# Azure/gpu-provisioner

Hardware: AMD Instinct MI355X
Metric: nodeclaims_per_min (higher is better)
Workload: dtype n/a; 1 GPU; model=MI355X NodeClaim provisioning (karpenter CloudProvider contract), vm_sku=Standard_ND128isr_MI355X_v6, concurrent_nodeclaims=8, cloud=in-memory fake AKS, zero latency (BASELINE config #1), apiserver=in-memory, server-side CRD validation on, cycle=create→Launched→Registered→Initialized(amd.com/gpu)→delete→gone, parallelism=single

## Files before the change

### gpu_provisioner_amd/fake/apiserver.py

```python
from __future__ import annotations

import asyncio
import os
from collections import deque
from collections import defaultdict
from typing import Any, AsyncIterator, Callable, Optional

from ..kube import objects as ko
from ..kube.client import (
    ADDED,
    DELETED,
    MODIFIED,
    AlreadyExistsError,
    APIError,
    ConflictError,
    GoneError,
    InvalidError,
    KubeClient,
    LabelSelector,
    NotFoundError,
    json_merge_patch,
    match_field_selector,
    merge_patch_owned,
)

_WATCH_HISTORY = 4096
_WATCH_BROKEN = "__WATCH_BROKEN__"
_EVENT_CAP = 20000

_native_revstore = None
if os.environ.get("GPU_PROVISIONER_PURE_PYTHON") != "1":
    try:
        from .._native import _revstore as _native_revstore
    except ImportError:
        _native_revstore = None
NATIVE_REVSTORE = _native_revstore is not None
if NATIVE_REVSTORE:
    _native_revstore.set_helpers(ko.uuid4_str, ko.now_rfc3339)

_SELECTABLE_FIELDS = {
    ("v1", "Pod"): {
        "spec.nodeName",
        "spec.schedulerName",
        "spec.restartPolicy",
        "spec.serviceAccountName",
        "spec.hostNetwork",
        "status.phase",
        "status.podIP",
        "status.nominatedNodeName",
    },
    ("v1", "Node"): {"spec.unschedulable"},
    ("v1", "Namespace"): {"status.phase", "name"},
    ("v1", "Secret"): {"type"},
    ("v1", "Event"): {
        "involvedObject.kind",
        "involvedObject.namespace",
        "involvedObject.name",
        "involvedObject.uid",
        "involvedObject.apiVersion",
        "involvedObject.resourceVersion",
        "involvedObject.fieldPath",
        "reason",
        "reportingComponent",
        "source",
        "type",
    },
}
_GENERIC_FIELDS = {"metadata.name", "metadata.namespace"}


def validate_field_selector(api_version: str, kind: str, selector: str) -> None:
    if not selector:
        return
    allowed = _GENERIC_FIELDS | _SELECTABLE_FIELDS.get((api_version, kind), set())
    for part in selector.split(","):
        part = part.strip()
        if not part:
            continue
        key = part.split("!=" if "!=" in part else "=", 1)[0].strip()
        if key not in allowed:
            raise InvalidError(f"field label not supported: {key}")


def _key(namespace: str, name: str) -> tuple:
    return (namespace or "", name)


def _gvk(api_version: str, kind: str) -> tuple:
    return (api_version, kind)


class InMemoryAPIServer:

    def __init__(self):
        self._store: dict = defaultdict(dict)
        self._rv = 0
        self._native = _native_revstore
        self._event_cap = _EVENT_CAP
        self._lock = asyncio.Lock()
        self._watchers: list = []
        self._history: deque = deque(maxlen=_WATCH_HISTORY)
        self.reactors: list = []
        self.validators: dict = {}
        self.eviction_reactor: Optional[Callable] = None
        self.evictions: list = []


    def _next_rv(self) -> str:
        self._rv += 1
        return str(self._rv)

    def _fire_reactors(self, verb: str, gvk: tuple, payload: Any) -> None:
        for r in list(self.reactors):
            err = r(verb, gvk, payload)
            if err is not None:
                raise err

    def _broadcast(self, gvk: tuple, event_type: str, obj: dict) -> None:
        self._history.append((self._rv, gvk, event_type, obj))
        for wgvk, queue in self._watchers:
            if wgvk == gvk:
                queue.put_nowait((event_type, obj))

    def _bump(self, obj: dict) -> None:
        obj["metadata"]["resourceVersion"] = self._next_rv()

    def _validate(self, gvk: tuple, new: dict, old: Optional[dict]) -> None:
        fn = self.validators.get(gvk)
        if fn is None:
            return
        errs = fn(new, old)
        if errs:
            raise InvalidError(
                f"{gvk[1]} {ko.name_of(new)} is invalid: " + "; ".join(errs[:5])
            )


    async def get(self, api_version: str, kind: str, name: str, namespace: str) -> dict:
        async with self._lock:
            gvk = (api_version, kind)
            if self.reactors:
                self._fire_reactors("get", gvk, name)
            if self._native is not None:
                out = self._native.get(self._store[gvk], namespace, name)
                if out is not NotImplemented:
                    return out
            obj = self._store[gvk].get(_key(namespace, name))
            if obj is None:
                raise NotFoundError(f"{kind} {namespace}/{name} not found")
            return ko.deep_copy(obj)

    async def list(
        self,
        api_version: str,
        kind: str,
        namespace: str,
        label_selector: str,
        field_selector: str,
    ) -> tuple:
        async with self._lock:
            gvk = _gvk(api_version, kind)
            validate_field_selector(api_version, kind, field_selector)
            self._fire_reactors("list", gvk, None)
            sel = LabelSelector.parse(label_selector) if label_selector else None
            out = []
            for (ns, _), obj in self._store[gvk].items():
                if namespace and ns != namespace:
                    continue
                if sel and not sel.matches(ko.labels_of(obj)):
                    continue
                if not match_field_selector(obj, field_selector):
                    continue
                out.append(ko.deep_copy(obj))
            return out, str(self._peek_rv())

    def _peek_rv(self) -> int:
        return self._rv

    async def create(self, obj: dict) -> dict:
        async with self._lock:
            api_version, kind = obj.get("apiVersion", ""), obj.get("kind", "")
            if not api_version or not kind or not ko.name_of(obj):
                raise InvalidError("apiVersion, kind and metadata.name are required")
            gvk = (api_version, kind)
            if self.reactors:
                self._fire_reactors("create", gvk, obj)
            if self._native is not None:
                out = self._native.create(
                    self, gvk, self._store[gvk], obj, self.validators.get(gvk), self._event_cap
                )
                if out is not NotImplemented:
                    return out
            key = _key(ko.namespace_of(obj), ko.name_of(obj))
            if key in self._store[gvk]:
                raise AlreadyExistsError(f"{kind} {key[0]}/{key[1]} already exists")
            stored = ko.deep_copy(obj)
            m = ko.meta(stored)
            m["uid"] = m.get("uid") or ko.uuid4_str()
            m["creationTimestamp"] = m.get("creationTimestamp") or ko.now_rfc3339()
            m["generation"] = 1
            self._validate(gvk, stored, None)
            self._bump(stored)
            self._store[gvk][key] = stored
            if kind == "Event" and len(self._store[gvk]) > self._event_cap:
                drop = next(iter(self._store[gvk]))
                del self._store[gvk][drop]
            self._broadcast(gvk, ADDED, stored)
            return ko.deep_copy(stored)

    async def update(self, obj: dict, subresource: str = "") -> dict:
        async with self._lock:
            api_version, kind = obj.get("apiVersion", ""), obj.get("kind", "")
            gvk = (api_version, kind)
            if self.reactors:
                self._fire_reactors("update", gvk, obj)
            if self._native is not None:
                out = self._native.update(
                    self, gvk, self._store[gvk], obj, subresource, self.validators.get(gvk)
                )
                if out is not NotImplemented:
                    return out
            key = _key(ko.namespace_of(obj), ko.name_of(obj))
            cur = self._store[gvk].get(key)
            if cur is None:
                raise NotFoundError(f"{kind} {key[0]}/{key[1]} not found")
            rv = obj.get("metadata", {}).get("resourceVersion")
            if rv and rv != cur["metadata"]["resourceVersion"]:
                raise ConflictError(
                    f"{kind} {key[1]}: resourceVersion mismatch ({rv} != {cur['metadata']['resourceVersion']})"
                )
            return self._apply_update(gvk, key, cur, obj, subresource)

    def _apply_update(
        self, gvk: tuple, key: tuple, cur: dict, obj: dict, subresource: str, owned: bool = False
    ) -> dict:
        if subresource == "status":
            stored = {**cur, "metadata": {**cur["metadata"]}}
            stored["status"] = ko.deep_copy(obj.get("status", {}))
        else:
            if ko.is_deleting(cur):
                added = set(ko.finalizers_of(obj)) - set(ko.finalizers_of(cur))
                if added:
                    raise InvalidError(
                        "metadata.finalizers: Forbidden: no new finalizers can "
                        f"be added if the object is being deleted (added: {sorted(added)})"
                    )
            new = obj if owned else ko.deep_copy(obj)
            new["status"] = cur.get("status", {})
            nm = ko.meta(new)
            cm = cur["metadata"]
            for f in ("uid", "creationTimestamp", "generation", "deletionTimestamp"):
                if f in cm:
                    nm[f] = cm[f]
                else:
                    nm.pop(f, None)
            ns, cs = new.get("spec"), cur.get("spec")
            if ns is cs:
                pass
            elif ns != cs:
                nm["generation"] = cm.get("generation", 1) + 1
            elif "spec" in new:
                new["spec"] = cs
            stored = new
        self._validate(gvk, stored, cur)
        self._bump(stored)
        if ko.is_deleting(stored) and not ko.finalizers_of(stored) and subresource != "status":
            del self._store[gvk][key]
            self._broadcast(gvk, DELETED, stored)
        else:
            self._store[gvk][key] = stored
            self._broadcast(gvk, MODIFIED, stored)
        return ko.deep_copy(stored)

    async def patch(
        self,
        api_version: str,
        kind: str,
        name: str,
        patch: dict,
        namespace: str,
        subresource: str,
    ) -> dict:
        async with self._lock:
            gvk = (api_version, kind)
            if self.reactors:
                self._fire_reactors("patch", gvk, name)
            if self._native is not None:
                out = self._native.patch(
                    self, gvk, self._store[gvk], namespace, name, patch, subresource,
                    self.validators.get(gvk),
                )
                if out is not NotImplemented:
                    return out
            key = _key(namespace, name)
            cur = self._store[gvk].get(key)
            if cur is None:
                raise NotFoundError(f"{kind} {namespace}/{name} not found")
            req_rv = (patch.get("metadata") or {}).get("resourceVersion")
            if req_rv and req_rv != cur["metadata"]["resourceVersion"]:
                raise ConflictError(
                    f"{kind} {name}: resourceVersion mismatch "
                    f"({req_rv} != {cur['metadata']['resourceVersion']})"
                )
            if subresource == "status":
                merged_status = json_merge_patch(cur.get("status", {}), patch.get("status", patch))
                return self._apply_update(gvk, key, cur, {"status": merged_status}, "status")
            merged = merge_patch_owned(cur, patch)
            merged.setdefault("metadata", {})["resourceVersion"] = cur["metadata"]["resourceVersion"]
            return self._apply_update(gvk, key, cur, merged, "", owned=True)

    async def delete(
        self,
        api_version: str,
        kind: str,
        name: str,
        namespace: str,
        uid_precondition: str = "",
        grace_period_seconds: Optional[int] = None,
    ) -> None:
        async with self._lock:
            gvk = (api_version, kind)
            if self.reactors:
                self._fire_reactors("delete", gvk, name)
            if self._native is not None:
                out = self._native.delete(
                    self, gvk, self._store[gvk], namespace, name, uid_precondition
                )
                if out is not NotImplemented:
                    return out
            key = _key(namespace, name)
            cur = self._store[gvk].get(key)
            if cur is None:
                raise NotFoundError(f"{kind} {namespace}/{name} not found")
            if uid_precondition and ko.uid_of(cur) != uid_precondition:
                raise ConflictError(f"{kind} {name}: uid precondition failed")
            if ko.finalizers_of(cur):
                if not ko.is_deleting(cur):
                    stored = {**cur, "metadata": {**cur["metadata"]}}
                    ko.meta(stored)["deletionTimestamp"] = ko.now_rfc3339()
                    self._bump(stored)
                    self._store[gvk][key] = stored
                    self._broadcast(gvk, MODIFIED, stored)
                return
            stored = {**cur, "metadata": {**cur["metadata"]}}
            ko.meta(stored)["deletionTimestamp"] = ko.now_rfc3339()
            self._bump(stored)
            del self._store[gvk][key]
            self._broadcast(gvk, DELETED, stored)

    async def evict(self, pod: dict, grace_period_seconds: Optional[int]) -> None:
        async with self._lock:
            if self.eviction_reactor is not None:
                err = self.eviction_reactor(pod)
                if err is not None:
                    raise err
            gvk = _gvk("v1", "Pod")
            key = _key(ko.namespace_of(pod), ko.name_of(pod))
            cur = self._store[gvk].get(key)
            if cur is None:
                raise NotFoundError(f"Pod {key[0]}/{key[1]} not found")
            self.evictions.append(key)
            stored = ko.deep_copy(cur)
            ko.meta(stored)["deletionTimestamp"] = ko.now_rfc3339()
            self._bump(stored)
            if ko.finalizers_of(cur):
                self._store[gvk][key] = stored
                self._broadcast(gvk, MODIFIED, stored)
            else:
                del self._store[gvk][key]
                self._broadcast(gvk, DELETED, stored)

    def subscribe(self, api_version: str, kind: str, resource_version: str) -> tuple:
        gvk = _gvk(api_version, kind)
        queue: asyncio.Queue = asyncio.Queue()
        if resource_version:
            rv = int(resource_version)
            if self._history:
                oldest = self._history[0][0]
                if rv + 1 < oldest and any(True for _ in self._store[gvk]):
                    raise GoneError(f"resourceVersion {rv} too old")
            for erv, egvk, etype, eobj in self._history:
                if egvk == gvk and erv > rv:
                    queue.put_nowait((etype, ko.deep_copy(eobj)))
        entry = (gvk, queue)
        self._watchers.append(entry)

        def unsubscribe():
            try:
                self._watchers.remove(entry)
            except ValueError:
                pass

        return queue, unsubscribe

    def break_watches(self) -> int:
        broken = 0
        for _, queue in list(self._watchers):
            queue.put_nowait((_WATCH_BROKEN, None))
            broken += 1
        return broken


class InMemoryClient(KubeClient):

    def __init__(self, server: InMemoryAPIServer):
        self.server = server

    async def get(self, api_version: str, kind: str, name: str, namespace: str = "") -> dict:
        return await self.server.get(api_version, kind, name, namespace)

    async def list(
        self,
        api_version: str,
        kind: str,
        namespace: str = "",
        label_selector: str = "",
        field_selector: str = "",
    ) -> list:
        items, _rv = await self.server.list(api_version, kind, namespace, label_selector, field_selector)
        return items

    async def list_with_rv(
        self,
        api_version: str,
        kind: str,
        namespace: str = "",
        label_selector: str = "",
        field_selector: str = "",
    ) -> tuple:
        return await self.server.list(api_version, kind, namespace, label_selector, field_selector)

    async def create(self, obj: dict) -> dict:
        return await self.server.create(obj)

    async def update(self, obj: dict) -> dict:
        return await self.server.update(obj)

    async def update_status(self, obj: dict) -> dict:
        return await self.server.update(obj, subresource="status")

    async def patch(
        self,
        api_version: str,
        kind: str,
        name: str,
        patch: dict,
        namespace: str = "",
        subresource: str = "",
    ) -> dict:
        return await self.server.patch(api_version, kind, name, patch, namespace, subresource)

    async def delete(
        self,
        api_version: str,
        kind: str,
        name: str,
        namespace: str = "",
        uid_precondition: str = "",
        grace_period_seconds: Optional[int] = None,
    ) -> None:
        await self.server.delete(
            api_version, kind, name, namespace, uid_precondition, grace_period_seconds
        )

    async def watch(
        self,
        api_version: str,
        kind: str,
        namespace: str = "",
        resource_version: str = "",
        label_selector: str = "",
    ) -> AsyncIterator[tuple]:
        queue, unsubscribe = self.server.subscribe(api_version, kind, resource_version)
        sel = LabelSelector.parse(label_selector) if label_selector else None
        try:
            while True:
                event_type, obj = await queue.get()
                if event_type == _WATCH_BROKEN:
                    raise APIError("watch stream broken")
                if namespace and ko.namespace_of(obj) != namespace:
                    continue
                if sel and not sel.matches(ko.labels_of(obj)):
                    continue
                yield event_type, obj
        finally:
            unsubscribe()

    async def evict(self, pod: dict, grace_period_seconds: Optional[int] = None) -> None:
        await self.server.evict(pod, grace_period_seconds)
```

### gpu_provisioner_amd/kube/crdschema.py

```python
from __future__ import annotations

import re
from typing import Optional

from .objects import _native_jsontree

_native_valid = _native_jsontree.crd_valid if _native_jsontree is not None else None


def _compile_schema(schema: dict, cache: Optional[dict] = None) -> dict:
    if cache is None:
        cache = {}
    sid = id(schema)
    if sid in cache:
        return cache[sid]
    out = dict(schema)
    cache[sid] = out
    if "pattern" in out:
        out["_pattern_re"] = re.compile(out["pattern"])
    if "enum" in out:
        out["_enum_set"] = frozenset(out["enum"])
    if "properties" in out:
        out["properties"] = {
            k: _compile_schema(v, cache) for k, v in out["properties"].items()
        }
    if isinstance(out.get("items"), dict):
        out["items"] = _compile_schema(out["items"], cache)
    if isinstance(out.get("additionalProperties"), dict):
        out["additionalProperties"] = _compile_schema(out["additionalProperties"], cache)
    for branch in ("anyOf", "oneOf", "allOf"):
        if branch in out:
            out[branch] = [_compile_schema(b, cache) for b in out[branch]]
    return out


def validate(obj, schema: dict, path: str = "$") -> list:
    errs: list = []
    _validate(obj, schema, (path,), errs)
    return errs


def _render(parts: tuple) -> str:
    return "".join(parts)


def _validate(obj, schema: dict, path: tuple, errs: list) -> None:
    t = schema.get("type")
    if t == "object" or ("properties" in schema and t is None):
        if not isinstance(obj, dict):
            errs.append(f"{_render(path)}: expected object, got {type(obj).__name__}")
            return
        props = schema.get("properties")
        ap = schema.get("additionalProperties")
        if props:
            extra_ok = schema.get("x-kubernetes-preserve-unknown-fields") or ap is not None
            for k, v in obj.items():
                sub = props.get(k)
                if sub is not None:
                    _validate(v, sub, path + (".", k), errs)
                elif isinstance(ap, dict):
                    _validate(v, ap, path + (".", k), errs)
                elif not extra_ok:
                    errs.append(f"{_render(path)}.{k}: unknown field")
        elif isinstance(ap, dict):
            for k, v in obj.items():
                _validate(v, ap, path + (".", k), errs)
        for req in schema.get("required", ()):
            if req not in obj:
                errs.append(f"{_render(path)}.{req}: required field missing")
    elif t == "array":
        if not isinstance(obj, list):
            errs.append(f"{_render(path)}: expected array, got {type(obj).__name__}")
            return
        if "maxItems" in schema and len(obj) > schema["maxItems"]:
            errs.append(
                f"{_render(path)}: {len(obj)} items exceeds maxItems {schema['maxItems']}"
            )
        items = schema.get("items")
        if items:
            for i, item in enumerate(obj):
                _validate(item, items, path + (f"[{i}]",), errs)
    elif t == "string":
        if not isinstance(obj, str):
            errs.append(f"{_render(path)}: expected string, got {type(obj).__name__}")
        else:
            enum_set = schema.get("_enum_set")
            if enum_set is not None:
                if obj not in enum_set:
                    errs.append(f"{_render(path)}: {obj!r} not in enum {schema['enum']}")
            elif "enum" in schema and obj not in schema["enum"]:
                errs.append(f"{_render(path)}: {obj!r} not in enum {schema['enum']}")
            pat = schema.get("_pattern_re")
            if pat is not None:
                if pat.search(obj) is None:
                    errs.append(
                        f"{_render(path)}: {obj!r} does not match pattern {schema['pattern']!r}"
                    )
            elif "pattern" in schema and re.search(schema["pattern"], obj) is None:
                errs.append(
                    f"{_render(path)}: {obj!r} does not match pattern {schema['pattern']!r}"
                )
            if "maxLength" in schema and len(obj) > schema["maxLength"]:
                errs.append(
                    f"{_render(path)}: length {len(obj)} exceeds maxLength {schema['maxLength']}"
                )
            if "minLength" in schema and len(obj) < schema["minLength"]:
                errs.append(
                    f"{_render(path)}: length {len(obj)} below minLength {schema['minLength']}"
                )
    elif t == "integer":
        if not isinstance(obj, int) or isinstance(obj, bool):
            errs.append(f"{_render(path)}: expected integer, got {type(obj).__name__}")
        else:
            if "minimum" in schema and obj < schema["minimum"]:
                errs.append(f"{_render(path)}: {obj} below minimum {schema['minimum']}")
            if "maximum" in schema and obj > schema["maximum"]:
                errs.append(f"{_render(path)}: {obj} above maximum {schema['maximum']}")
    elif t == "boolean":
        if not isinstance(obj, bool):
            errs.append(f"{_render(path)}: expected boolean, got {type(obj).__name__}")
    if "anyOf" in schema:
        branch_errs: list = []
        ok = False
        for b in schema["anyOf"]:
            merged = b
            if b.get("type") == "string" and any(
                f in schema for f in ("pattern", "_pattern_re", "maxLength", "minLength", "enum")
            ):
                merged = {**b}
                for f in ("pattern", "_pattern_re", "maxLength", "minLength", "enum", "_enum_set"):
                    if f in schema:
                        merged[f] = schema[f]
            be: list = []
            _validate(obj, merged, path, be)
            if not be:
                ok = True
                break
            if not branch_errs:
                branch_errs = be
        if not ok:
            errs.append(
                f"{_render(path)}: no anyOf branch matched ({'; '.join(branch_errs[:1])})"
            )


_MISSING = object()


def _validate_changed(new, old, schema: dict, path: str, errs: list) -> None:
    if new is old:
        return
    props = schema.get("properties")
    if isinstance(new, dict) and isinstance(old, dict) and props is not None:
        ap = schema.get("additionalProperties")
        extra_ok = schema.get("x-kubernetes-preserve-unknown-fields") or ap is not None
        for k, v in new.items():
            sub = props.get(k)
            if sub is None and isinstance(ap, dict):
                sub = ap
            if sub is None:
                if props and not extra_ok:
                    errs.append(f"{path}.{k}: unknown field")
                continue
            ov = old.get(k, _MISSING)
            if ov is _MISSING:
                _validate(v, sub, (path, ".", k), errs)
            else:
                _validate_changed(v, ov, sub, f"{path}.{k}", errs)
        for req in schema.get("required", ()):
            if req not in new:
                errs.append(f"{path}.{req}: required field missing")
        return
    items = schema.get("items")
    if isinstance(new, list) and isinstance(old, list) and isinstance(items, dict):
        if "maxItems" in schema and len(new) > schema["maxItems"]:
            errs.append(f"{path}: {len(new)} items exceeds maxItems {schema['maxItems']}")
        for i, item in enumerate(new):
            if any(item is o or item == o for o in old):
                continue
            _validate(item, items, (path, f"[{i}]"), errs)
        return
    if new == old:
        return
    _validate(new, schema, (path,), errs)


def _apply_defaults(obj, schema: dict) -> None:
    if not isinstance(obj, dict):
        return
    for name, sub in (schema.get("properties") or {}).items():
        if name not in obj and "default" in sub:
            obj[name] = sub["default"]
        if name in obj:
            if isinstance(obj[name], dict):
                _apply_defaults(obj[name], sub)
            elif isinstance(obj[name], list) and isinstance(sub.get("items"), dict):
                for item in obj[name]:
                    _apply_defaults(item, sub["items"])


class CRDValidator:

    def __init__(self, crd: dict):
        versions = crd["spec"]["versions"]
        assert len(versions) == 1
        self.schema = _compile_schema(versions[0]["schema"]["openAPIV3Schema"])
        spec_schema = self.schema.get("properties", {}).get("spec", {})
        self.spec_immutable = any(
            r.get("rule") == "self == oldSelf"
            for r in spec_schema.get("x-kubernetes-validations", [])
        )

    @classmethod
    def from_file(cls, path: str) -> "CRDValidator":
        import yaml

        return cls(next(yaml.safe_load_all(open(path))))

    def __call__(self, new: dict, old: Optional[dict]) -> list:
        if old is None:
            _apply_defaults(new, self.schema)
        if _native_valid is not None and _native_valid(
            self.schema, new, old, self.spec_immutable
        ):
            return []
        return self._violations(new, old)

    def _violations(self, new: dict, old: Optional[dict]) -> list:
        errs: list = []
        if old is None:
            errs += validate(new, self.schema)
        else:
            props = self.schema.get("properties", {})
            for key in ("spec", "status"):
                ns, olds = new.get(key), old.get(key)
                sub = props.get(key)
                if sub is not None and ns is not None:
                    _validate_changed(ns, olds, sub, f"$.{key}", errs)
            if self.spec_immutable:
                ns, olds = new.get("spec"), old.get("spec")
                if ns is not olds and ns != olds:
                    errs.append("$.spec: spec is immutable (CEL: self == oldSelf)")
        ref = (new.get("spec") or {}).get("nodeClassRef")
        if isinstance(ref, dict):
            for f in ("group", "kind", "name"):
                if f in ref and ref[f] == "":
                    errs.append(f"$.spec.nodeClassRef.{f}: may not be empty (CEL)")
        return errs
```

### native/jsontree.cpp

```cpp
#define PY_SSIZE_T_CLEAN
#include <Python.h>

#include "jsontree_walk.h"

namespace {

using jsontree_walk::copy_tree;
using jsontree_walk::merge;
using jsontree_walk::merge_owned;

PyObject* py_deep_copy(PyObject*, PyObject* obj) { return copy_tree(obj); }

PyObject* py_json_merge_patch(PyObject*, PyObject* const* args, Py_ssize_t nargs) {
    if (nargs != 2) {
        PyErr_SetString(PyExc_TypeError, "json_merge_patch(target, patch) takes 2 arguments");
        return nullptr;
    }
    return merge(args[0], args[1], false);
}

PyObject* str_metadata;

PyObject* py_merge_patch_owned(PyObject*, PyObject* const* args, Py_ssize_t nargs) {
    if (nargs != 2) {
        PyErr_SetString(PyExc_TypeError, "merge_patch_owned(cur, patch) takes 2 arguments");
        return nullptr;
    }
    return merge_owned(args[0], args[1], str_metadata);
}


struct Names {
    PyObject *type, *properties, *additionalProperties, *preserve, *required, *items,
        *maxItems, *enum_set, *enum_, *pattern_re, *pattern, *maxLength, *minLength,
        *minimum, *maximum, *anyOf, *search, *spec, *status, *nodeClassRef, *group,
        *kind, *name, *empty;
} S;

inline PyObject* sget(PyObject* schema, PyObject* key) {
    PyObject* v = PyDict_GetItemWithError(schema, key);
    if (v == nullptr) PyErr_Clear();
    return v;
}

inline PyObject* sget2(PyObject* schema, PyObject* overlay, PyObject* key) {
    if (overlay != nullptr) {
        PyObject* v = sget(overlay, key);
        if (v != nullptr) return v;
    }
    return sget(schema, key);
}

inline bool is_str(PyObject* o, const char* s) {
    return o != nullptr && PyUnicode_CheckExact(o) && PyUnicode_CompareWithASCIIString(o, s) == 0;
}

int len_cmp(Py_ssize_t n, PyObject* limit, int op) {
    PyObject* pn = PyLong_FromSsize_t(n);
    if (pn == nullptr) return -1;
    int r = PyObject_RichCompareBool(pn, limit, op);
    Py_DECREF(pn);
    return r;
}

int validate(PyObject* obj, PyObject* schema, PyObject* overlay);

int validate_changed(PyObject* nw, PyObject* old, PyObject* schema);

int check_required(PyObject* obj, PyObject* schema) {
    PyObject* req = sget(schema, S.required);
    if (req == nullptr) return 1;
    if (!PyList_CheckExact(req) && !PyTuple_CheckExact(req)) return 0;
    Py_ssize_t n = PySequence_Fast_GET_SIZE(req);
    for (Py_ssize_t i = 0; i < n; i++) {
        int has = PyDict_Contains(obj, PySequence_Fast_GET_ITEM(req, i));
        if (has <= 0) return has;
    }
    return 1;
}

int validate_string(PyObject* obj, PyObject* schema, PyObject* overlay) {
    if (!PyUnicode_Check(obj)) return 0;
    if (!PyUnicode_CheckExact(obj)) return 0;
    PyObject* enum_set = sget2(schema, overlay, S.enum_set);
    if (enum_set != nullptr && enum_set != Py_None) {
        int in = PySequence_Contains(enum_set, obj);
        if (in <= 0) return in;
    } else {
        PyObject* en = sget2(schema, overlay, S.enum_);
        if (en != nullptr) {
            int in = PySequence_Contains(en, obj);
            if (in <= 0) return in;
        }
    }
    PyObject* pat = sget2(schema, overlay, S.pattern_re);
    if (pat != nullptr && pat != Py_None) {
        PyObject* m = PyObject_CallMethodOneArg(pat, S.search, obj);
        if (m == nullptr) return -1;
        bool miss = m == Py_None;
        Py_DECREF(m);
        if (miss) return 0;
    } else if (sget2(schema, overlay, S.pattern) != nullptr) {
        return 0;
    }
    PyObject* lim = sget2(schema, overlay, S.maxLength);
    if (lim != nullptr) {
        int r = len_cmp(PyUnicode_GET_LENGTH(obj), lim, Py_GT);
        if (r != 0) return r < 0 ? -1 : 0;
    }
    lim = sget2(schema, overlay, S.minLength);
    if (lim != nullptr) {
        int r = len_cmp(PyUnicode_GET_LENGTH(obj), lim, Py_LT);
        if (r != 0) return r < 0 ? -1 : 0;
    }
    return 1;
}

int validate_object(PyObject* obj, PyObject* schema) {
    if (!PyDict_Check(obj)) return 0;
    if (!PyDict_CheckExact(obj)) return 0;
    PyObject* props = sget(schema, S.properties);
    PyObject* ap = sget(schema, S.additionalProperties);
    if (ap == Py_None) ap = nullptr;
    if (ap != nullptr && PyDict_Check(ap) && !PyDict_CheckExact(ap)) return 0;
    bool ap_schema = ap != nullptr && PyDict_CheckExact(ap);
    int props_true = props == nullptr ? 0 : PyObject_IsTrue(props);
    if (props_true < 0) return -1;
    if (props_true && !PyDict_CheckExact(props)) return 0;
    if (props_true || ap_schema) {
        bool extra_ok = ap != nullptr;
        if (props_true && !extra_ok) {
            PyObject* pu = sget(schema, S.preserve);
            int t = pu == nullptr ? 0 : PyObject_IsTrue(pu);
            if (t < 0) return -1;
            extra_ok = t != 0;
        }
        Py_ssize_t pos = 0;
        PyObject *k, *v;
        while (PyDict_Next(obj, &pos, &k, &v)) {
            PyObject* sub = nullptr;
            if (props_true) {
                sub = PyDict_GetItemWithError(props, k);
                if (sub == nullptr && PyErr_Occurred()) return -1;
                if (sub == Py_None) sub = nullptr;
            }
            if (sub == nullptr && ap_schema) sub = ap;
            if (sub == nullptr) {
                if (!extra_ok) return 0;
                continue;
            }
            if (!PyDict_CheckExact(sub)) return 0;
            int r = validate(v, sub, nullptr);
            if (r <= 0) return r;
        }
    }
    return check_required(obj, schema);
}

int validate_any_of(PyObject* obj, PyObject* schema, PyObject* branches) {
    if (!PyList_CheckExact(branches)) return 0;
    bool string_fields = sget(schema, S.pattern) || sget(schema, S.pattern_re) ||
                         sget(schema, S.maxLength) || sget(schema, S.minLength) ||
                         sget(schema, S.enum_);
    for (Py_ssize_t i = 0; i < PyList_GET_SIZE(branches); i++) {
        PyObject* b = PyList_GET_ITEM(branches, i);
        if (!PyDict_CheckExact(b)) return 0;
        PyObject* overlay = nullptr;
        if (string_fields && is_str(sget(b, S.type), "string")) overlay = schema;
        int r = validate(obj, b, overlay);
        if (r != 0) return r;
    }
    return 0;
}

int validate(PyObject* obj, PyObject* schema, PyObject* overlay) {
    if (Py_EnterRecursiveCall(" while validating against a CRD schema")) return -1;
    int r = 1;
    PyObject* t = sget(schema, S.type);
    if (t != nullptr && t != Py_None && !PyUnicode_CheckExact(t)) {
        r = 0;
    } else if (is_str(t, "object") ||
               ((t == nullptr || t == Py_None) && sget(schema, S.properties) != nullptr)) {
        r = validate_object(obj, schema);
    } else if (is_str(t, "array")) {
        if (!PyList_CheckExact(obj)) {
            r = 0;
        } else {
            PyObject* lim = sget(schema, S.maxItems);
            if (lim != nullptr) {
                int c = len_cmp(PyList_GET_SIZE(obj), lim, Py_GT);
                if (c != 0) r = c < 0 ? -1 : 0;
            }
            PyObject* items = sget(schema, S.items);
            int items_true = (r == 1 && items != nullptr) ? PyObject_IsTrue(items) : 0;
            if (items_true < 0) r = -1;
            if (r == 1 && items_true) {
                if (!PyDict_CheckExact(items)) r = 0;
                for (Py_ssize_t i = 0; r == 1 && i < PyList_GET_SIZE(obj); i++)
                    r = validate(PyList_GET_ITEM(obj, i), items, nullptr);
            }
        }
    } else if (is_str(t, "string")) {
        r = validate_string(obj, schema, overlay);
    } else if (is_str(t, "integer")) {
        if (!PyLong_Check(obj) || PyBool_Check(obj)) {
            r = 0;
        } else {
            PyObject* lim = sget(schema, S.minimum);
            if (lim != nullptr) {
                int c = PyObject_RichCompareBool(obj, lim, Py_LT);
                if (c != 0) r = c < 0 ? -1 : 0;
            }
            lim = sget(schema, S.maximum);
            if (r == 1 && lim != nullptr) {
                int c = PyObject_RichCompareBool(obj, lim, Py_GT);
                if (c != 0) r = c < 0 ? -1 : 0;
            }
        }
    } else if (is_str(t, "boolean")) {
        if (!PyBool_Check(obj)) r = 0;
    }
    if (r == 1) {
        PyObject* any_of = sget(schema, S.anyOf);
        if (any_of != nullptr)
            r = overlay != nullptr ? 0 : validate_any_of(obj, schema, any_of);
    }
    Py_LeaveRecursiveCall();
    return r;
}

int validate_changed(PyObject* nw, PyObject* old, PyObject* schema) {
    if (nw == old) return 1;
    if (Py_EnterRecursiveCall(" while validating against a CRD schema")) return -1;
    int r = 1;
    PyObject* props = sget(schema, S.properties);
    if (props == Py_None) props = nullptr;
    PyObject* items = sget(schema, S.items);
    if ((PyDict_Check(nw) && !PyDict_CheckExact(nw)) || (PyDict_Check(old) && !PyDict_CheckExact(old)) ||
        (PyList_Check(nw) && !PyList_CheckExact(nw)) || (PyList_Check(old) && !PyList_CheckExact(old)) ||
        (props != nullptr && !PyDict_CheckExact(props)) ||
        (items != nullptr && PyDict_Check(items) && !PyDict_CheckExact(items))) {
        r = 0;
    } else if (PyDict_CheckExact(nw) && PyDict_CheckExact(old) && props != nullptr) {
        PyObject* ap = sget(schema, S.additionalProperties);
        if (ap == Py_None) ap = nullptr;
        bool ap_schema = ap != nullptr && PyDict_CheckExact(ap);
        if (ap != nullptr && PyDict_Check(ap) && !ap_schema) r = 0;
        bool extra_ok = ap != nullptr;
        if (r == 1 && !extra_ok) {
            PyObject* pu = sget(schema, S.preserve);
            int t = pu == nullptr ? 0 : PyObject_IsTrue(pu);
            if (t < 0) r = -1;
            extra_ok = t > 0;
        }
        bool props_true = PyDict_GET_SIZE(props) > 0;
        Py_ssize_t pos = 0;
        PyObject *k, *v;
        while (r == 1 && PyDict_Next(nw, &pos, &k, &v)) {
            PyObject* sub = PyDict_GetItemWithError(props, k);
            if (sub == nullptr && PyErr_Occurred()) { r = -1; break; }
            if (sub == Py_None) sub = nullptr;
            if (sub == nullptr && ap_schema) sub = ap;
            if (sub == nullptr) {
                if (props_true && !extra_ok) r = 0;
                continue;
            }
            if (!PyDict_CheckExact(sub)) { r = 0; break; }
            PyObject* ov = PyDict_GetItemWithError(old, k);
            if (ov == nullptr && PyErr_Occurred()) { r = -1; break; }
            r = ov == nullptr ? validate(v, sub, nullptr) : validate_changed(v, ov, sub);
        }
        if (r == 1) r = check_required(nw, schema);
    } else if (PyList_CheckExact(nw) && PyList_CheckExact(old) && items != nullptr &&
               PyDict_CheckExact(items)) {
        PyObject* lim = sget(schema, S.maxItems);
        if (lim != nullptr) {
            int c = len_cmp(PyList_GET_SIZE(nw), lim, Py_GT);
            if (c != 0) r = c < 0 ? -1 : 0;
        }
        for (Py_ssize_t i = 0; r == 1 && i < PyList_GET_SIZE(nw); i++) {
            PyObject* item = PyList_GET_ITEM(nw, i);
            Py_INCREF(item);
            int seen = 0;
            for (Py_ssize_t j = 0; seen == 0 && j < PyList_GET_SIZE(old); j++) {
                PyObject* o = PyList_GET_ITEM(old, j);
                Py_INCREF(o);
                seen = PyObject_RichCompareBool(item, o, Py_EQ);
                Py_DECREF(o);
            }
            if (seen < 0) r = -1;
            else if (seen == 0) r = validate(item, items, nullptr);
            Py_DECREF(item);
        }
    } else {
        int eq = PyObject_RichCompareBool(nw, old, Py_EQ);
        if (eq < 0) r = -1;
        else if (eq == 0) r = validate(nw, schema, nullptr);
    }
    Py_LeaveRecursiveCall();
    return r;
}

int crd_valid(PyObject* schema, PyObject* nw, PyObject* old, bool spec_immutable) {
    if (!PyDict_CheckExact(schema) || !PyDict_CheckExact(nw)) return 0;
    PyObject* spec = sget(nw, S.spec);
    if (old == Py_None) {
        int r = validate(nw, schema, nullptr);
        if (r <= 0) return r;
    } else {
        if (!PyDict_CheckExact(old)) return 0;
        PyObject* props = sget(schema, S.properties);
        if (props != nullptr && !PyDict_CheckExact(props)) return 0;
        PyObject* keys[2] = {S.spec, S.status};
        for (PyObject* key : keys) {
            PyObject* ns = sget(nw, key);
            PyObject* olds = sget(old, key);
            PyObject* sub = props ? sget(props, key) : nullptr;
            if (sub == nullptr || sub == Py_None || ns == nullptr || ns == Py_None) continue;
            if (!PyDict_CheckExact(sub)) return 0;
            int r = validate_changed(ns, olds ? olds : Py_None, sub);
            if (r <= 0) return r;
        }
        if (spec_immutable) {
            PyObject* ns = spec ? spec : Py_None;
            PyObject* olds = sget(old, S.spec);
            if (olds == nullptr) olds = Py_None;
            if (ns != olds) {
                int ne = PyObject_RichCompareBool(ns, olds, Py_NE);
                if (ne != 0) return ne < 0 ? -1 : 0;
            }
        }
    }
    if (spec == nullptr) return 1;
    int spec_true = PyObject_IsTrue(spec);
    if (spec_true < 0) return -1;
    if (!spec_true) return 1;
    if (!PyDict_CheckExact(spec)) return 0;
    PyObject* ref = sget(spec, S.nodeClassRef);
    if (ref == nullptr || !PyDict_Check(ref)) return 1;
    if (!PyDict_CheckExact(ref)) return 0;
    PyObject* fields[3] = {S.group, S.kind, S.name};
    for (PyObject* f : fields) {
        PyObject* v = sget(ref, f);
        if (v == nullptr) continue;
        int eq = PyObject_RichCompareBool(v, S.empty, Py_EQ);
        if (eq != 0) return eq < 0 ? -1 : 0;
    }
    return 1;
}

PyObject* py_crd_valid(PyObject*, PyObject* const* args, Py_ssize_t nargs) {
    if (nargs != 4) {
        PyErr_SetString(PyExc_TypeError,
                        "crd_valid(schema, new, old_or_None, spec_immutable) takes 4 arguments");
        return nullptr;
    }
    int imm = PyObject_IsTrue(args[3]);
    if (imm < 0) return nullptr;
    int r = crd_valid(args[0], args[1], args[2], imm != 0);
    if (r < 0) {
        PyErr_Clear();
        r = 0;
    }
    return PyBool_FromLong(r);
}

PyMethodDef methods[] = {
    {"deep_copy", (PyCFunction)py_deep_copy, METH_O,
     "deep_copy(obj): copy exact dict/list recursively, share everything else."},
    {"json_merge_patch", (PyCFunction)(void (*)(void))py_json_merge_patch, METH_FASTCALL,
     "json_merge_patch(target, patch): RFC 7386 merge patch, returning a new dict."},
    {"merge_patch_owned", (PyCFunction)(void (*)(void))py_merge_patch_owned, METH_FASTCALL,
     "merge_patch_owned(cur, patch): == deep_copy(json_merge_patch(cur, patch)), "
     "sharing the subtrees of cur the patch does not touch."},
    {"crd_valid", (PyCFunction)(void (*)(void))py_crd_valid, METH_FASTCALL,
     "crd_valid(schema, new, old_or_None, spec_immutable): True when CRDValidator "
     "would report no violation."},
    {nullptr, nullptr, 0, nullptr},
};

PyModuleDef moduledef = {
    PyModuleDef_HEAD_INIT, "_jsontree",
    "Native JSON-tree copy, merge patch and CRD validation fast path.", -1, methods,
    nullptr, nullptr, nullptr, nullptr,
};

bool intern_names() {
    struct { PyObject** slot; const char* text; } table[] = {
        {&str_metadata, "metadata"},
        {&S.type, "type"},
        {&S.properties, "properties"},
        {&S.additionalProperties, "additionalProperties"},
        {&S.preserve, "x-kubernetes-preserve-unknown-fields"},
        {&S.required, "required"},
        {&S.items, "items"},
        {&S.maxItems, "maxItems"},
        {&S.enum_set, "_enum_set"},
        {&S.enum_, "enum"},
        {&S.pattern_re, "_pattern_re"},
        {&S.pattern, "pattern"},
        {&S.maxLength, "maxLength"},
        {&S.minLength, "minLength"},
        {&S.minimum, "minimum"},
        {&S.maximum, "maximum"},
        {&S.anyOf, "anyOf"},
        {&S.search, "search"},
        {&S.spec, "spec"},
        {&S.status, "status"},
        {&S.nodeClassRef, "nodeClassRef"},
        {&S.group, "group"},
        {&S.kind, "kind"},
        {&S.name, "name"},
        {&S.empty, ""},
    };
    for (auto& e : table) {
        *e.slot = PyUnicode_InternFromString(e.text);
        if (*e.slot == nullptr) return false;
    }
    return true;
}

}

PyMODINIT_FUNC PyInit__jsontree(void) {
    if (!intern_names()) return nullptr;
    return PyModule_Create(&moduledef);
}
```

### native/revstore.cpp

```cpp
#define PY_SSIZE_T_CLEAN
#include <Python.h>

#include <limits.h>

#include "jsontree_walk.h"

namespace {

using jsontree_walk::copy_tree;
using jsontree_walk::merge;
using jsontree_walk::merge_owned;

struct Names {
    PyObject *metadata, *name, *namespace_, *uid, *creationTimestamp, *generation,
        *deletionTimestamp, *finalizers, *resourceVersion, *spec, *status, *empty, *Event,
        *ADDED, *MODIFIED, *DELETED, *rv_attr, *history_attr, *watchers_attr, *append,
        *put_nowait;
} S;

PyObject* long_one;
PyObject* uuid4_str;
PyObject* now_rfc3339;

struct Ref {
    PyObject* p;
    explicit Ref(PyObject* o = nullptr) : p(o) {}
    ~Ref() { Py_XDECREF(p); }
    Ref(const Ref&) = delete;
    Ref& operator=(const Ref&) = delete;
    void reset(PyObject* o) { Py_XSETREF(p, o); }
    PyObject* release() {
        PyObject* o = p;
        p = nullptr;
        return o;
    }
    operator PyObject*() const { return p; }
};

inline PyObject* newref(PyObject* o) {
    Py_XINCREF(o);
    return o;
}

inline PyObject* miss() { Py_RETURN_NOTIMPLEMENTED; }

inline int look(PyObject* d, PyObject* key, PyObject** out) {
    *out = PyDict_GetItemWithError(d, key);
    if (*out != nullptr) return 1;
    return PyErr_Occurred() ? -1 : 0;
}

inline int truthy(PyObject* d, PyObject* key) {
    PyObject* v;
    int r = look(d, key, &v);
    if (r <= 0) return r;
    Ref hold(newref(v));
    return PyObject_IsTrue(v);
}

inline bool str_eq(PyObject* a, PyObject* b) {
    return a == b || PyUnicode_Compare(a, b) == 0;
}

PyObject* make_key(PyObject* ns, PyObject* name) {
    if (ns == nullptr || ns == Py_None) ns = S.empty;
    if (name == nullptr || !PyUnicode_CheckExact(ns) || !PyUnicode_CheckExact(name)) return nullptr;
    return PyTuple_Pack(2, ns, name);
}

int current(PyObject* bucket, PyObject* key, PyObject** cur, PyObject** cm) {
    int r = look(bucket, key, cur);
    if (r <= 0) return r;
    if (!PyDict_CheckExact(*cur)) return 0;
    r = look(*cur, S.metadata, cm);
    if (r == 1 && !PyDict_CheckExact(*cm)) return 0;
    return r;
}

int rv_precondition(PyObject* meta, PyObject* cm) {
    PyObject* want = nullptr;
    if (meta != nullptr && look(meta, S.resourceVersion, &want) < 0) return -1;
    if (want == nullptr || want == Py_None) return 1;
    if (!PyUnicode_CheckExact(want)) return 0;
    if (PyUnicode_GET_LENGTH(want) == 0) return 1;
    PyObject* have;
    int r = look(cm, S.resourceVersion, &have);
    if (r <= 0) return r;
    return PyUnicode_CheckExact(have) && str_eq(want, have);
}

int no_new_finalizers(PyObject* nm, PyObject* cm) {
    PyObject *nf, *cf;
    if (look(nm, S.finalizers, &nf) < 0 || look(cm, S.finalizers, &cf) < 0) return -1;
    if (nf == nullptr || nf == Py_None) return 1;
    if (cf == Py_None) cf = nullptr;
    if (!PyList_CheckExact(nf) || (cf != nullptr && !PyList_CheckExact(cf))) return 0;
    for (Py_ssize_t i = 0; i < PyList_GET_SIZE(nf); i++) {
        PyObject* f = PyList_GET_ITEM(nf, i);
        if (!PyUnicode_CheckExact(f)) return 0;
        bool found = false;
        for (Py_ssize_t j = 0; !found && cf != nullptr && j < PyList_GET_SIZE(cf); j++) {
            PyObject* c = PyList_GET_ITEM(cf, j);
            if (!PyUnicode_CheckExact(c)) return 0;
            found = str_eq(f, c);
        }
        if (!found) return 0;
    }
    return 1;
}

int valid(PyObject* validator, PyObject* nw, PyObject* old) {
    if (validator == Py_None) return 1;
    PyObject* args[2] = {nw, old};
    Ref errs(PyObject_Vectorcall(validator, args, 2, nullptr));
    if (errs == nullptr) return -1;
    int t = PyObject_IsTrue(errs);
    return t < 0 ? -1 : !t;
}


struct Sink {
    Ref append;
    Ref watchers;
    long long rv = 0;
};

int open_sink(PyObject* server, Sink& s) {
    Ref rv(PyObject_GetAttr(server, S.rv_attr));
    Ref hist(rv != nullptr ? PyObject_GetAttr(server, S.history_attr) : nullptr);
    if (hist != nullptr) s.append.reset(PyObject_GetAttr(hist, S.append));
    if (s.append != nullptr) s.watchers.reset(PyObject_GetAttr(server, S.watchers_attr));
    if (s.watchers == nullptr) {
        PyErr_Clear();
        return 0;
    }
    PyObject* ws = s.watchers.p;
    if (!PyLong_CheckExact(rv.p) || !PyList_CheckExact(ws)) return 0;
    int overflow = 0;
    s.rv = PyLong_AsLongLongAndOverflow(rv.p, &overflow);
    if (overflow || s.rv < 0 || s.rv == LLONG_MAX) return 0;
    for (Py_ssize_t i = 0; i < PyList_GET_SIZE(ws); i++) {
        PyObject* w = PyList_GET_ITEM(ws, i);
        if (!PyTuple_CheckExact(w) || PyTuple_GET_SIZE(w) != 2) return 0;
    }
    return 1;
}

int commit(PyObject* server, Sink& s, PyObject* gvk, PyObject* bucket, PyObject* key,
           PyObject* stored, PyObject* nm, PyObject* event_type, bool remove,
           Py_ssize_t cap = -1) {
    long long n = s.rv + 1;
    Ref rv_str(PyUnicode_FromFormat("%lld", n));
    Ref rv_int(PyLong_FromLongLong(n));
    if (rv_str == nullptr || rv_int == nullptr) return -1;
    Ref entry(PyTuple_Pack(4, (PyObject*)rv_int, gvk, event_type, stored));
    Ref event(PyTuple_Pack(2, event_type, stored));
    if (entry == nullptr || event == nullptr) return -1;
    if (PyDict_SetItem(nm, S.resourceVersion, rv_str) < 0) return -1;
    if (PyObject_SetAttr(server, S.rv_attr, rv_int) < 0) return -1;
    if ((remove ? PyDict_DelItem(bucket, key) : PyDict_SetItem(bucket, key, stored)) < 0) return -1;
    if (cap >= 0 && PyDict_GET_SIZE(bucket) > cap) {
        Py_ssize_t pos = 0;
        PyObject *k, *v;
        if (PyDict_Next(bucket, &pos, &k, &v)) {
            Ref oldest(newref(k));
            if (PyDict_DelItem(bucket, oldest) < 0) return -1;
        }
    }
    Ref appended(PyObject_CallOneArg(s.append, entry));
    if (appended == nullptr) return -1;
    PyObject* ws = s.watchers.p;
    for (Py_ssize_t i = 0; i < PyList_GET_SIZE(ws); i++) {
        PyObject* w = PyList_GET_ITEM(ws, i);
        if (!PyTuple_CheckExact(w) || PyTuple_GET_SIZE(w) != 2) continue;
        Ref hold(newref(w));
        int eq = PyObject_RichCompareBool(PyTuple_GET_ITEM(w, 0), gvk, Py_EQ);
        if (eq < 0) return -1;
        if (!eq) continue;
        Ref put(PyObject_CallMethodOneArg(PyTuple_GET_ITEM(w, 1), S.put_nowait, event));
        if (put == nullptr) return -1;
    }
    return 0;
}


enum Mode {
    STATUS,
    STATUS_OWNED,
    MAIN,
    MAIN_OWNED,
};

PyObject* apply_update(PyObject* server, PyObject* gvk, PyObject* bucket, PyObject* key,
                       PyObject* cur, PyObject* cm, PyObject* obj, Mode mode,
                       PyObject* validator) {
    Sink sink;
    if (!open_sink(server, sink)) return miss();
    Ref stored, meta_ref;
    bool remove = false;
    if (mode == STATUS || mode == STATUS_OWNED) {
        stored.reset(PyDict_Copy(cur));
        meta_ref.reset(PyDict_Copy(cm));
        if (stored == nullptr || meta_ref == nullptr) return nullptr;
        Ref status;
        if (mode == STATUS_OWNED) {
            status.reset(newref(obj));
        } else {
            PyObject* v;
            if (look(obj, S.status, &v) < 0) return nullptr;
            status.reset(v != nullptr ? copy_tree(v) : PyDict_New());
        }
        if (status == nullptr || PyDict_SetItem(stored, S.metadata, meta_ref) < 0 ||
            PyDict_SetItem(stored, S.status, status) < 0)
            return nullptr;
    } else {
        PyObject* om;
        int r = look(obj, S.metadata, &om);
        if (r < 0) return nullptr;
        if (r == 0 || !PyDict_CheckExact(om)) return miss();
        int deleting = truthy(cm, S.deletionTimestamp);
        if (deleting < 0) return nullptr;
        if (deleting) {
            r = no_new_finalizers(om, cm);
            if (r < 0) return nullptr;
            if (r == 0) return miss();
        }
        stored.reset(mode == MAIN_OWNED ? newref(obj) : copy_tree(obj));
        if (stored == nullptr) return nullptr;
        PyObject* v;
        if (look(cur, S.status, &v) < 0) return nullptr;
        Ref status(v != nullptr ? newref(v) : PyDict_New());
        if (status == nullptr || PyDict_SetItem(stored, S.status, status) < 0) return nullptr;
        if (look(stored, S.metadata, &v) <= 0) return nullptr;
        meta_ref.reset(newref(v));
        PyObject* fixed[4] = {S.uid, S.creationTimestamp, S.generation, S.deletionTimestamp};
        for (PyObject* f : fixed) {
            if (look(cm, f, &v) < 0) return nullptr;
            if (v != nullptr) {
                if (PyDict_SetItem(meta_ref, f, v) < 0) return nullptr;
            } else {
                int has = PyDict_Contains(meta_ref, f);
                if (has < 0 || (has && PyDict_DelItem(meta_ref, f) < 0)) return nullptr;
            }
        }
        PyObject *ns, *cs;
        if (look(stored, S.spec, &ns) < 0 || look(cur, S.spec, &cs) < 0) return nullptr;
        PyObject* a = ns != nullptr ? ns : Py_None;
        PyObject* b = cs != nullptr ? cs : Py_None;
        if (a != b) {
            int ne = PyObject_RichCompareBool(a, b, Py_NE);
            if (ne < 0) return nullptr;
            if (ne) {
                PyObject* gen;
                if (look(cm, S.generation, &gen) < 0) return nullptr;
                if (gen == nullptr) gen = long_one;
                if (!PyLong_CheckExact(gen)) return miss();
                Ref next(PyNumber_Add(gen, long_one));
                if (next == nullptr || PyDict_SetItem(meta_ref, S.generation, next) < 0) return nullptr;
            } else if (ns != nullptr && cs != nullptr) {
                if (PyDict_SetItem(stored, S.spec, cs) < 0) return nullptr;
            }
        }
    }
    int ok = valid(validator, stored, cur);
    if (ok < 0) return nullptr;
    if (!ok) return miss();
    if (mode == MAIN || mode == MAIN_OWNED) {
        int deleting = truthy(meta_ref, S.deletionTimestamp);
        int fins = deleting > 0 ? truthy(meta_ref, S.finalizers) : 0;
        if (deleting < 0 || fins < 0) return nullptr;
        remove = deleting && !fins;
    }
    if (commit(server, sink, gvk, bucket, key, stored, meta_ref, remove ? S.DELETED : S.MODIFIED,
               remove) < 0)
        return nullptr;
    return copy_tree(stored);
}

inline bool is_gvk(PyObject* gvk) { return PyTuple_CheckExact(gvk) && PyTuple_GET_SIZE(gvk) == 2; }

inline int subresource_mode(PyObject* sub) {
    if (!PyUnicode_CheckExact(sub)) return -1;
    if (PyUnicode_GET_LENGTH(sub) == 0) return MAIN;
    return str_eq(sub, S.status) ? STATUS : -1;
}


PyObject* py_get(PyObject*, PyObject* const* args, Py_ssize_t nargs) {
    if (nargs != 3) {
        PyErr_SetString(PyExc_TypeError, "get(bucket, namespace, name) takes 3 arguments");
        return nullptr;
    }
    if (!PyDict_Check(args[0])) return miss();
    Ref key(make_key(args[1], args[2]));
    if (key == nullptr) return PyErr_Occurred() ? nullptr : miss();
    PyObject* obj;
    int r = look(args[0], key, &obj);
    if (r < 0) return nullptr;
    if (r == 0) return miss();
    return copy_tree(obj);
}

PyObject* py_create(PyObject*, PyObject* const* args, Py_ssize_t nargs) {
    if (nargs != 6) {
        PyErr_SetString(PyExc_TypeError,
                        "create(server, gvk, bucket, obj, validator, event_cap) takes 6 arguments");
        return nullptr;
    }
    PyObject *server = args[0], *gvk = args[1], *bucket = args[2], *obj = args[3],
             *validator = args[4];
    Py_ssize_t cap = PyLong_AsSsize_t(args[5]);
    if (cap == -1 && PyErr_Occurred()) return nullptr;
    if (!is_gvk(gvk) || !PyDict_Check(bucket) || !PyDict_CheckExact(obj) || uuid4_str == nullptr)
        return miss();
    PyObject* om;
    int r = look(obj, S.metadata, &om);
    if (r < 0) return nullptr;
    if (r == 0 || !PyDict_CheckExact(om)) return miss();
    PyObject *name, *ns;
    if (look(om, S.name, &name) < 0 || look(om, S.namespace_, &ns) < 0) return nullptr;
    if (name == nullptr || !PyUnicode_CheckExact(name) || PyUnicode_GET_LENGTH(name) == 0)
        return miss();
    Ref key(make_key(ns, name));
    if (key == nullptr) return PyErr_Occurred() ? nullptr : miss();
    r = PyDict_Contains(bucket, key);
    if (r < 0) return nullptr;
    if (r) return miss();
    Sink sink;
    if (!open_sink(server, sink)) return miss();

    Ref stored(copy_tree(obj));
    if (stored == nullptr) return nullptr;
    PyObject* m;
    if (look(stored, S.metadata, &m) <= 0) return nullptr;
    Ref meta_ref(newref(m));
    struct { PyObject* key; PyObject* make; } fill[2] = {
        {S.uid, uuid4_str}, {S.creationTimestamp, now_rfc3339}};
    for (auto& f : fill) {
        int has = truthy(meta_ref, f.key);
        if (has < 0) return nullptr;
        if (has) continue;
        Ref v(PyObject_CallNoArgs(f.make));
        if (v == nullptr || PyDict_SetItem(meta_ref, f.key, v) < 0) return nullptr;
    }
    if (PyDict_SetItem(meta_ref, S.generation, long_one) < 0) return nullptr;
    int ok = valid(validator, stored, Py_None);
    if (ok < 0) return nullptr;
    if (!ok) return miss();
    PyObject* kind = PyTuple_GET_ITEM(gvk, 1);
    bool capped = PyUnicode_CheckExact(kind) && str_eq(kind, S.Event);
    if (commit(server, sink, gvk, bucket, key, stored, meta_ref, S.ADDED, false,
               capped ? cap : -1) < 0)
        return nullptr;
    return copy_tree(stored);
}

PyObject* py_update(PyObject*, PyObject* const* args, Py_ssize_t nargs) {
    if (nargs != 6) {
        PyErr_SetString(PyExc_TypeError,
                        "update(server, gvk, bucket, obj, subresource, validator) takes 6 arguments");
        return nullptr;
    }
    PyObject *server = args[0], *gvk = args[1], *bucket = args[2], *obj = args[3];
    int mode = subresource_mode(args[4]);
    if (mode < 0 || !is_gvk(gvk) || !PyDict_Check(bucket) || !PyDict_CheckExact(obj)) return miss();
    PyObject* om;
    int r = look(obj, S.metadata, &om);
    if (r < 0) return nullptr;
    if (r == 0 || !PyDict_CheckExact(om)) return miss();
    PyObject *name, *ns;
    if (look(om, S.name, &name) < 0 || look(om, S.namespace_, &ns) < 0) return nullptr;
    Ref key(make_key(ns, name));
    if (key == nullptr) return PyErr_Occurred() ? nullptr : miss();
    PyObject *cur, *cm;
    r = current(bucket, key, &cur, &cm);
    if (r < 0) return nullptr;
    if (r == 0) return miss();
    Ref hold_cur(newref(cur)), hold_cm(newref(cm));
    r = rv_precondition(om, cm);
    if (r < 0) return nullptr;
    if (r == 0) return miss();
    return apply_update(server, gvk, bucket, key, cur, cm, obj, (Mode)mode, args[5]);
}

PyObject* py_patch(PyObject*, PyObject* const* args, Py_ssize_t nargs) {
    if (nargs != 8) {
        PyErr_SetString(PyExc_TypeError,
                        "patch(server, gvk, bucket, namespace, name, patch, subresource, validator) "
                        "takes 8 arguments");
        return nullptr;
    }
    PyObject *server = args[0], *gvk = args[1], *bucket = args[2], *patch = args[5];
    int mode = subresource_mode(args[6]);
    if (mode < 0 || !is_gvk(gvk) || !PyDict_Check(bucket) || !PyDict_CheckExact(patch)) return miss();
    Ref key(make_key(args[3], args[4]));
    if (key == nullptr) return PyErr_Occurred() ? nullptr : miss();
    PyObject *cur, *cm;
    int r = current(bucket, key, &cur, &cm);
    if (r < 0) return nullptr;
    if (r == 0) return miss();
    Ref hold_cur(newref(cur)), hold_cm(newref(cm));
    PyObject* pm;
    r = look(patch, S.metadata, &pm);
    if (r < 0) return nullptr;
    if (r == 1 && !PyDict_CheckExact(pm)) return miss();
    r = rv_precondition(pm, cm);
    if (r < 0) return nullptr;
    if (r == 0) return miss();
    if (mode == STATUS) {
        PyObject *sp, *cs;
        if (look(patch, S.status, &sp) < 0 || look(cur, S.status, &cs) < 0) return nullptr;
        Ref merged(merge(cs, sp != nullptr ? sp : patch, true));
        if (merged == nullptr) return nullptr;
        return apply_update(server, gvk, bucket, key, cur, cm, merged, STATUS_OWNED, args[7]);
    }
    PyObject* rv;
    r = look(cm, S.resourceVersion, &rv);
    if (r < 0) return nullptr;
    if (r == 0) return miss();
    Ref merged(merge_owned(cur, patch, S.metadata));
    if (merged == nullptr) return nullptr;
    PyObject* mm;
    r = PyDict_CheckExact(merged.p) ? look(merged, S.metadata, &mm) : 0;
    if (r < 0) return nullptr;
    if (r == 0 || !PyDict_CheckExact(mm)) return miss();
    if (PyDict_SetItem(mm, S.resourceVersion, rv) < 0) return nullptr;
    return apply_update(server, gvk, bucket, key, cur, cm, merged, MAIN_OWNED, args[7]);
}

PyObject* py_delete(PyObject*, PyObject* const* args, Py_ssize_t nargs) {
    if (nargs != 6) {
        PyErr_SetString(PyExc_TypeError,
                        "delete(server, gvk, bucket, namespace, name, uid_precondition) takes 6 arguments");
        return nullptr;
    }
    PyObject *server = args[0], *gvk = args[1], *bucket = args[2], *want_uid = args[5];
    if (!is_gvk(gvk) || !PyDict_Check(bucket) || !PyUnicode_CheckExact(want_uid) ||
        now_rfc3339 == nullptr)
        return miss();
    Ref key(make_key(args[3], args[4]));
    if (key == nullptr) return PyErr_Occurred() ? nullptr : miss();
    PyObject *cur, *cm;
    int r = current(bucket, key, &cur, &cm);
    if (r < 0) return nullptr;
    if (r == 0) return miss();
    Ref hold_cur(newref(cur)), hold_cm(newref(cm));
    if (PyUnicode_GET_LENGTH(want_uid) > 0) {
        PyObject* uid;
        if (look(cm, S.uid, &uid) < 0) return nullptr;
        if (uid == nullptr) uid = S.empty;
        if (!PyUnicode_CheckExact(uid) || !str_eq(uid, want_uid)) return miss();
    }
    int fins = truthy(cm, S.finalizers);
    int deleting = fins > 0 ? truthy(cm, S.deletionTimestamp) : 0;
    if (fins < 0 || deleting < 0) return nullptr;
    if (fins && deleting) Py_RETURN_NONE;
    Sink sink;
    if (!open_sink(server, sink)) return miss();
    Ref stored(PyDict_Copy(cur)), nm(PyDict_Copy(cm));
    Ref now(PyObject_CallNoArgs(now_rfc3339));
    if (stored == nullptr || nm == nullptr || now == nullptr ||
        PyDict_SetItem(stored, S.metadata, nm) < 0 ||
        PyDict_SetItem(nm, S.deletionTimestamp, now) < 0)
        return nullptr;
    if (commit(server, sink, gvk, bucket, key, stored, nm, fins ? S.MODIFIED : S.DELETED, !fins) < 0)
        return nullptr;
    Py_RETURN_NONE;
}

PyObject* py_set_helpers(PyObject*, PyObject* const* args, Py_ssize_t nargs) {
    if (nargs != 2 || !PyCallable_Check(args[0]) || !PyCallable_Check(args[1])) {
        PyErr_SetString(PyExc_TypeError, "set_helpers(uuid4_str, now_rfc3339) takes two callables");
        return nullptr;
    }
    Py_XSETREF(uuid4_str, newref(args[0]));
    Py_XSETREF(now_rfc3339, newref(args[1]));
    Py_RETURN_NONE;
}

#define FAST(f) (PyCFunction)(void (*)(void))f, METH_FASTCALL

PyMethodDef methods[] = {
    {"set_helpers", FAST(py_set_helpers),
     "set_helpers(uuid4_str, now_rfc3339): bind the uid and clock functions create and delete call."},
    {"get", FAST(py_get), "get(bucket, namespace, name): a copy of the stored revision."},
    {"create", FAST(py_create),
     "create(server, gvk, bucket, obj, validator, event_cap): store a new object, return a copy."},
    {"update", FAST(py_update),
     "update(server, gvk, bucket, obj, subresource, validator): replace the main resource or the "
     "status, return a copy."},
    {"patch", FAST(py_patch),
     "patch(server, gvk, bucket, namespace, name, patch, subresource, validator): merge patch the "
     "main resource or the status, return a copy."},
    {"delete", FAST(py_delete),
     "delete(server, gvk, bucket, namespace, name, uid_precondition): mark deleting or remove."},
    {nullptr, nullptr, 0, nullptr},
};

PyModuleDef moduledef = {
    PyModuleDef_HEAD_INIT, "_revstore",
    "Native success path of the in-memory apiserver's verbs; every entry point returns "
    "NotImplemented, with nothing touched, for what the Python body has to handle.",
    -1, methods, nullptr, nullptr, nullptr, nullptr,
};

bool intern_names() {
    struct { PyObject** slot; const char* text; } table[] = {
        {&S.metadata, "metadata"},
        {&S.name, "name"},
        {&S.namespace_, "namespace"},
        {&S.uid, "uid"},
        {&S.creationTimestamp, "creationTimestamp"},
        {&S.generation, "generation"},
        {&S.deletionTimestamp, "deletionTimestamp"},
        {&S.finalizers, "finalizers"},
        {&S.resourceVersion, "resourceVersion"},
        {&S.spec, "spec"},
        {&S.status, "status"},
        {&S.empty, ""},
        {&S.Event, "Event"},
        {&S.ADDED, "ADDED"},
        {&S.MODIFIED, "MODIFIED"},
        {&S.DELETED, "DELETED"},
        {&S.rv_attr, "_rv"},
        {&S.history_attr, "_history"},
        {&S.watchers_attr, "_watchers"},
        {&S.append, "append"},
        {&S.put_nowait, "put_nowait"},
    };
    for (auto& e : table) {
        *e.slot = PyUnicode_InternFromString(e.text);
        if (*e.slot == nullptr) return false;
    }
    long_one = PyLong_FromLong(1);
    return long_one != nullptr;
}

}

PyMODINIT_FUNC PyInit__revstore(void) {
    if (!intern_names()) return nullptr;
    return PyModule_Create(&moduledef);
}
```

Baseline: 113,300 NodeClaims/min.

## Precompile CRD schemas into native node trees and validate inside revstore verbs

Adds a C++ schema compiler that turns each CRD's OpenAPI schema into a tree of typed nodes with interned keys, hashes and parsed limits, held in a capsule on the validator. Validation and defaulting then walk this compiled tree instead of doing dict lookups on the schema every call, and defaulting moves into native code. The native revstore verbs also recognise CRDValidator instances and run the compiled walk directly, skipping the Python __call__ round trip. The cost is a second implementation of the schema semantics in C++ that must stay in step with the Python one. A standalone checker compares the native and Python results on a test corpus.

```diff
diff --git a/gpu_provisioner_amd/fake/apiserver.py b/gpu_provisioner_amd/fake/apiserver.py
--- a/gpu_provisioner_amd/fake/apiserver.py
+++ b/gpu_provisioner_amd/fake/apiserver.py
@@ -36,7 +36,10 @@
         _native_revstore = None
 NATIVE_REVSTORE = _native_revstore is not None
 if NATIVE_REVSTORE:
+    from ..kube import crdschema as _crdschema
+
     _native_revstore.set_helpers(ko.uuid4_str, ko.now_rfc3339)
+    _native_revstore.set_admission(_crdschema.CRDValidator, vars(_crdschema))
 
 _SELECTABLE_FIELDS = {
     ("v1", "Pod"): {
diff --git a/gpu_provisioner_amd/kube/crdschema.py b/gpu_provisioner_amd/kube/crdschema.py
--- a/gpu_provisioner_amd/kube/crdschema.py
+++ b/gpu_provisioner_amd/kube/crdschema.py
@@ -210,6 +210,11 @@
             r.get("rule") == "self == oldSelf"
             for r in spec_schema.get("x-kubernetes-validations", [])
         )
+        self._compiled = (
+            _native_jsontree.crd_compile(self.schema, self.spec_immutable)
+            if _native_jsontree is not None
+            else None
+        )
 
     @classmethod
     def from_file(cls, path: str) -> "CRDValidator":
@@ -218,6 +223,12 @@
         return cls(next(yaml.safe_load_all(open(path))))
 
     def __call__(self, new: dict, old: Optional[dict]) -> list:
+        if _native_valid is not None and self._compiled is not None:
+            if old is None:
+                _native_jsontree.crd_defaults(self._compiled, new)
+            if _native_jsontree.crd_valid_compiled(self._compiled, new, old):
+                return []
+            return self._violations(new, old)
         if old is None:
             _apply_defaults(new, self.schema)
         if _native_valid is not None and _native_valid(
diff --git a/hack/crdschema_walk_check.cpp b/hack/crdschema_walk_check.cpp
--- /dev/null
+++ b/hack/crdschema_walk_check.cpp
@@ -0,0 +1,107 @@
+#include "../native/crdschema_walk.h"
+
+#include <cstdio>
+#include <cstdlib>
+#include <cstring>
+
+namespace cw = crdschema_walk;
+
+static PyObject* must(PyObject* o, const char* what) {
+    if (o == nullptr) {
+        PyErr_Print();
+        std::fprintf(stderr, "failed: %s\n", what);
+        std::exit(2);
+    }
+    return o;
+}
+
+int main(int argc, char** argv) {
+    setenv("GPU_PROVISIONER_PURE_PYTHON", "1", 1);
+    Py_Initialize();
+    PyObject* sys_path = must(PySys_GetObject("path"), "sys.path");
+    PyObject* root = must(PyUnicode_FromString(argc > 1 ? argv[1] : "."), "root");
+    PyList_Insert(sys_path, 0, root);
+    if (!cw::init_names()) return 2;
+
+    PyObject* mod = must(PyImport_ImportModule("tests.test_native_admission"), "import corpus");
+    PyObject* copy = must(PyImport_ImportModule("copy"), "import copy");
+    PyObject* crdschema = must(PyImport_ImportModule("gpu_provisioner_amd.kube.crdschema"), "import crdschema");
+    PyObject* validators = must(PyObject_CallMethod(mod, "make_validators", nullptr), "validators");
+    PyObject* corpus = must(PyObject_CallMethod(mod, "corpus", nullptr), "corpus");
+
+    std::unordered_map<PyObject*, std::unique_ptr<cw::Schema>> compiled;
+    Py_ssize_t pos = 0;
+    PyObject *name, *validator;
+    while (PyDict_Next(validators, &pos, &name, &validator)) {
+        PyObject* schema = must(PyObject_GetAttrString(validator, "schema"), "schema");
+        PyObject* imm = must(PyObject_GetAttrString(validator, "spec_immutable"), "spec_immutable");
+        compiled[validator] = cw::compile(schema, PyObject_IsTrue(imm) == 1);
+        if (compiled[validator] == nullptr) {
+            std::fprintf(stderr, "schema %s did not compile\n", PyUnicode_AsUTF8(name));
+            return 1;
+        }
+        for (int i = 0; i < 1000; i++)
+            if (cw::compile(schema, false) == nullptr) return 1;
+        Py_DECREF(schema);
+        Py_DECREF(imm);
+    }
+    PyObject* raw = must(Py_BuildValue("{s:s,s:{s:{s:s,s:s}}}", "type", "object", "properties", "a",
+                                       "type", "string", "pattern", "^x"), "raw schema");
+    if (cw::compile(raw, false) != nullptr || PyErr_Occurred()) return 1;
+
+    long valid = 0, invalid = 0, deferred = 0, wrong = 0;
+    for (Py_ssize_t i = 0; i < PyList_GET_SIZE(corpus); i++) {
+        PyObject* row = PyList_GET_ITEM(corpus, i);
+        const char* label = PyUnicode_AsUTF8(PyTuple_GET_ITEM(row, 0));
+        validator = must(PyDict_GetItemWithError(validators, PyTuple_GET_ITEM(row, 1)), "validator");
+        const cw::Schema& schema = *compiled[validator];
+        PyObject* old = PyTuple_GET_ITEM(row, 3);
+        PyObject* nw = PyTuple_GET_ITEM(row, 2);
+        PyObject* mine = old == Py_None ? must(PyObject_CallMethod(copy, "deepcopy", "O", nw), "copy") : (Py_INCREF(nw), nw);
+        PyObject* theirs = old == Py_None ? must(PyObject_CallMethod(copy, "deepcopy", "O", nw), "copy") : (Py_INCREF(nw), nw);
+        if (old == Py_None) {
+            if (cw::apply_defaults(mine, schema.root) < 0) must(nullptr, "apply_defaults");
+            PyObject* vs = must(PyObject_GetAttrString(validator, "schema"), "schema");
+            Py_DECREF(must(PyObject_CallMethod(crdschema, "_apply_defaults", "OO", theirs, vs), "python defaults"));
+            Py_DECREF(vs);
+            PyObject* a = must(PyObject_CallMethod(mod, "ordered", "O", mine), "ordered");
+            PyObject* b = must(PyObject_CallMethod(mod, "ordered", "O", theirs), "ordered");
+            if (PyObject_RichCompareBool(a, b, Py_EQ) != 1) {
+                std::fprintf(stderr, "defaults differ: %s\n", label);
+                wrong++;
+            }
+            Py_DECREF(a);
+            Py_DECREF(b);
+        }
+        int r = cw::verdict(schema, mine, old);
+        if (r < 0) PyErr_Clear();
+        PyObject* errs = PyObject_CallMethod(validator, "_violations", "OO", theirs, old);
+        if (errs == nullptr) {
+            PyErr_Clear();
+            if (r > 0) wrong++;
+            deferred++;
+        } else {
+            bool want = PyList_GET_SIZE(errs) == 0;
+            bool subclass = std::strstr(label, "subclass:") != nullptr;
+            if (subclass ? (r > 0 && !want) : ((r > 0) != want)) {
+                std::fprintf(stderr, "verdict %d, python %s: %s\n", r, want ? "valid" : "invalid", label);
+                wrong++;
+            }
+            (r > 0 ? valid : invalid)++;
+            Py_DECREF(errs);
+        }
+        Py_DECREF(mine);
+        Py_DECREF(theirs);
+    }
+    std::printf("crdschema_walk_check: %ld inputs: %ld valid, %ld not valid, %ld python-raises, %ld wrong\n",
+                (long)PyList_GET_SIZE(corpus), valid, invalid, deferred, wrong);
+    compiled.clear();
+    Py_DECREF(raw);
+    Py_DECREF(corpus);
+    Py_DECREF(validators);
+    Py_DECREF(copy);
+    Py_DECREF(crdschema);
+    Py_DECREF(mod);
+    if (Py_FinalizeEx() < 0) return 2;
+    return wrong == 0 && valid > 50 && invalid > 50 ? 0 : 1;
+}
diff --git a/native/crdschema_walk.h b/native/crdschema_walk.h
--- /dev/null
+++ b/native/crdschema_walk.h
@@ -0,0 +1,624 @@
+#ifndef GPU_PROVISIONER_AMD_CRDSCHEMA_WALK_H
+#define GPU_PROVISIONER_AMD_CRDSCHEMA_WALK_H
+
+#define PY_SSIZE_T_CLEAN
+#include <Python.h>
+
+#include <memory>
+#include <unordered_map>
+#include <vector>
+
+namespace crdschema_walk {
+
+static const char* const CAPSULE_NAME = "gpu_provisioner_amd._native.crdschema";
+
+struct Names {
+    PyObject *type, *properties, *additionalProperties, *preserve, *required, *items,
+        *maxItems, *enum_set, *enum_, *pattern_re, *pattern, *maxLength, *minLength,
+        *minimum, *maximum, *anyOf, *default_, *search, *spec, *status, *nodeClassRef,
+        *group, *kind, *name, *empty;
+};
+static Names N;
+
+static inline bool init_names() {
+    struct { PyObject** slot; const char* text; } table[] = {
+        {&N.type, "type"},
+        {&N.properties, "properties"},
+        {&N.additionalProperties, "additionalProperties"},
+        {&N.preserve, "x-kubernetes-preserve-unknown-fields"},
+        {&N.required, "required"},
+        {&N.items, "items"},
+        {&N.maxItems, "maxItems"},
+        {&N.enum_set, "_enum_set"},
+        {&N.enum_, "enum"},
+        {&N.pattern_re, "_pattern_re"},
+        {&N.pattern, "pattern"},
+        {&N.maxLength, "maxLength"},
+        {&N.minLength, "minLength"},
+        {&N.minimum, "minimum"},
+        {&N.maximum, "maximum"},
+        {&N.anyOf, "anyOf"},
+        {&N.default_, "default"},
+        {&N.search, "search"},
+        {&N.spec, "spec"},
+        {&N.status, "status"},
+        {&N.nodeClassRef, "nodeClassRef"},
+        {&N.group, "group"},
+        {&N.kind, "kind"},
+        {&N.name, "name"},
+        {&N.empty, ""},
+    };
+    for (auto& e : table) {
+        *e.slot = PyUnicode_InternFromString(e.text);
+        if (*e.slot == nullptr) return false;
+    }
+    return true;
+}
+
+
+enum Type : unsigned char {
+    T_NONE,
+    T_OBJECT,
+    T_ARRAY,
+    T_STRING,
+    T_INTEGER,
+    T_BOOLEAN,
+    T_OTHER,
+};
+
+struct Limit {
+    bool present = false;
+    bool in_c = false;
+    long long c = 0;
+    PyObject* obj = nullptr;
+};
+
+struct Node;
+
+struct Prop {
+    PyObject* key;
+    Py_hash_t hash;
+    const Node* node;
+};
+
+struct Node {
+    Type type = T_NONE;
+    bool has_props = false;
+    bool ap_present = false;
+    bool preserve = false;
+    bool has_any_of = false;
+    bool has_default = false;
+    std::vector<Prop> props;
+    std::vector<PyObject*> required;
+    const Node* ap = nullptr;
+    const Node* items = nullptr;
+    Limit max_items, min_length, max_length, minimum, maximum;
+    PyObject* enum_set = nullptr;
+    PyObject* search = nullptr;
+    std::vector<const Node*> any_of;
+    PyObject* default_value = nullptr;
+};
+
+struct Schema {
+    std::vector<std::unique_ptr<Node>> nodes;
+    std::vector<PyObject*> held;
+    const Node* root = nullptr;
+    const Node* spec = nullptr;
+    const Node* status = nullptr;
+    bool spec_immutable = false;
+    Schema() = default;
+    Schema(const Schema&) = delete;
+    Schema& operator=(const Schema&) = delete;
+    ~Schema() {
+        for (PyObject* o : held) Py_DECREF(o);
+    }
+};
+
+static inline const Node* find_prop(const Node* n, PyObject* k) {
+    for (const Prop& p : n->props)
+        if (p.key == k) return p.node;
+    Py_hash_t h = PyObject_Hash(k);
+    for (const Prop& p : n->props)
+        if (p.hash == h && PyUnicode_Compare(p.key, k) == 0) return p.node;
+    return nullptr;
+}
+
+
+struct Compiler {
+    Schema& s;
+    std::unordered_map<PyObject*, Node*> memo;
+
+    explicit Compiler(Schema& schema) : s(schema) {}
+
+    PyObject* hold(PyObject* o) {
+        Py_INCREF(o);
+        s.held.push_back(o);
+        return o;
+    }
+
+    static PyObject* get(PyObject* schema, PyObject* key) {
+        PyObject* v = PyDict_GetItemWithError(schema, key);
+        if (v == nullptr) PyErr_Clear();
+        return v;
+    }
+
+    static PyObject* get2(PyObject* schema, PyObject* overlay, PyObject* key) {
+        if (overlay != nullptr) {
+            PyObject* v = get(overlay, key);
+            if (v != nullptr) return v;
+        }
+        return get(schema, key);
+    }
+
+    static bool is_str(PyObject* o, const char* text) {
+        return o != nullptr && PyUnicode_CheckExact(o) &&
+               PyUnicode_CompareWithASCIIString(o, text) == 0;
+    }
+
+    void limit(Limit& l, PyObject* v) {
+        if (v == nullptr) return;
+        l.present = true;
+        l.obj = hold(v);
+        if (PyLong_CheckExact(v)) {
+            int overflow = 0;
+            l.c = PyLong_AsLongLongAndOverflow(v, &overflow);
+            l.in_c = overflow == 0;
+        }
+    }
+
+    Node* node(PyObject* schema, PyObject* overlay) {
+        if (!PyDict_CheckExact(schema)) return nullptr;
+        if (overlay == nullptr) {
+            auto hit = memo.find(schema);
+            if (hit != memo.end()) return hit->second;
+        }
+        if (Py_EnterRecursiveCall(" while compiling a CRD schema")) return nullptr;
+        s.nodes.emplace_back(new Node());
+        Node* n = s.nodes.back().get();
+        if (overlay == nullptr) memo[schema] = n;
+        bool ok = fill(n, schema, overlay);
+        Py_LeaveRecursiveCall();
+        return ok ? n : nullptr;
+    }
+
+    bool fill(Node* n, PyObject* schema, PyObject* overlay) {
+        PyObject* t = get(schema, N.type);
+        if (t == nullptr || t == Py_None) {
+            int has = PyDict_Contains(schema, N.properties);
+            if (has < 0) return false;
+            n->type = has ? T_OBJECT : T_NONE;
+        } else if (!PyUnicode_CheckExact(t)) {
+            return false;
+        } else {
+            n->type = is_str(t, "object") ? T_OBJECT
+                    : is_str(t, "array") ? T_ARRAY
+                    : is_str(t, "string") ? T_STRING
+                    : is_str(t, "integer") ? T_INTEGER
+                    : is_str(t, "boolean") ? T_BOOLEAN
+                                           : T_OTHER;
+        }
+
+        PyObject* props = get(schema, N.properties);
+        if (props != nullptr && props != Py_None) {
+            if (!PyDict_CheckExact(props)) return false;
+            n->has_props = true;
+            Py_ssize_t pos = 0;
+            PyObject *k, *v;
+            while (PyDict_Next(props, &pos, &k, &v)) {
+                if (!PyUnicode_CheckExact(k)) return false;
+                const Node* sub = node(v, nullptr);
+                if (sub == nullptr) return false;
+                Py_INCREF(k);
+                PyUnicode_InternInPlace(&k);
+                s.held.push_back(k);
+                Py_hash_t h = PyObject_Hash(k);
+                if (h == -1) return false;
+                n->props.push_back({k, h, sub});
+            }
+        }
+
+        PyObject* ap = get(schema, N.additionalProperties);
+        if (ap != nullptr && ap != Py_None) {
+            n->ap_present = true;
+            if (PyDict_Check(ap)) {
+                n->ap = node(ap, nullptr);
+                if (n->ap == nullptr) return false;
+            }
+        }
+        PyObject* pu = get(schema, N.preserve);
+        if (pu != nullptr) {
+            int truth = PyObject_IsTrue(pu);
+            if (truth < 0) return false;
+            n->preserve = truth != 0;
+        }
+
+        PyObject* req = get(schema, N.required);
+        if (req != nullptr) {
+            if (!PyList_CheckExact(req) && !PyTuple_CheckExact(req)) return false;
+            for (Py_ssize_t i = 0; i < PySequence_Fast_GET_SIZE(req); i++)
+                n->required.push_back(hold(PySequence_Fast_GET_ITEM(req, i)));
+        }
+
+        PyObject* items = get(schema, N.items);
+        if (items != nullptr) {
+            if (PyDict_Check(items)) {
+                n->items = node(items, nullptr);
+                if (n->items == nullptr) return false;
+            } else {
+                int truth = PyObject_IsTrue(items);
+                if (truth != 0) return false;
+            }
+        }
+        limit(n->max_items, get(schema, N.maxItems));
+
+        PyObject* es = get2(schema, overlay, N.enum_set);
+        if (es == nullptr || es == Py_None) es = get2(schema, overlay, N.enum_);
+        if (es != nullptr) n->enum_set = hold(es);
+        PyObject* pat = get2(schema, overlay, N.pattern_re);
+        if (pat != nullptr && pat != Py_None) {
+            n->search = PyObject_GetAttr(pat, N.search);
+            if (n->search == nullptr) return false;
+            s.held.push_back(n->search);
+        } else if (get2(schema, overlay, N.pattern) != nullptr) {
+            return false;
+        }
+        limit(n->max_length, get2(schema, overlay, N.maxLength));
+        limit(n->min_length, get2(schema, overlay, N.minLength));
+
+        limit(n->minimum, get(schema, N.minimum));
+        limit(n->maximum, get(schema, N.maximum));
+
+        PyObject* any_of = get(schema, N.anyOf);
+        if (any_of != nullptr) {
+            if (overlay != nullptr || !PyList_CheckExact(any_of)) return false;
+            n->has_any_of = true;
+            bool string_fields = get(schema, N.pattern) || get(schema, N.pattern_re) ||
+                                 get(schema, N.maxLength) || get(schema, N.minLength) ||
+                                 get(schema, N.enum_);
+            for (Py_ssize_t i = 0; i < PyList_GET_SIZE(any_of); i++) {
+                PyObject* b = PyList_GET_ITEM(any_of, i);
+                if (!PyDict_CheckExact(b)) return false;
+                bool over = string_fields && is_str(get(b, N.type), "string");
+                const Node* branch = node(b, over ? schema : nullptr);
+                if (branch == nullptr) return false;
+                n->any_of.push_back(branch);
+            }
+        }
+
+        PyObject* dflt = get(schema, N.default_);
+        if (dflt != nullptr) {
+            n->has_default = true;
+            n->default_value = hold(dflt);
+        }
+        return true;
+    }
+};
+
+static inline std::unique_ptr<Schema> compile(PyObject* schema, bool spec_immutable) {
+    std::unique_ptr<Schema> s(new Schema());
+    Compiler c(*s);
+    s->root = c.node(schema, nullptr);
+    if (s->root == nullptr) {
+        PyErr_Clear();
+        return nullptr;
+    }
+    s->spec_immutable = spec_immutable;
+    if (s->root->has_props) {
+        s->spec = find_prop(s->root, N.spec);
+        s->status = find_prop(s->root, N.status);
+    }
+    return s;
+}
+
+static inline void capsule_free(PyObject* capsule) {
+    delete static_cast<Schema*>(PyCapsule_GetPointer(capsule, CAPSULE_NAME));
+}
+
+static inline PyObject* compile_capsule(PyObject* schema, bool spec_immutable) {
+    std::unique_ptr<Schema> s = compile(schema, spec_immutable);
+    if (s == nullptr) return nullptr;
+    PyObject* capsule = PyCapsule_New(s.get(), CAPSULE_NAME, capsule_free);
+    if (capsule != nullptr) s.release();
+    return capsule;
+}
+
+static inline const Schema* from_capsule(PyObject* o) {
+    if (o == nullptr || !PyCapsule_CheckExact(o) || !PyCapsule_IsValid(o, CAPSULE_NAME))
+        return nullptr;
+    return static_cast<const Schema*>(PyCapsule_GetPointer(o, CAPSULE_NAME));
+}
+
+
+static inline int len_beyond(Py_ssize_t n, const Limit& l, int op) {
+    if (l.in_c) return op == Py_GT ? n > l.c : n < l.c;
+    PyObject* pn = PyLong_FromSsize_t(n);
+    if (pn == nullptr) return -1;
+    int r = PyObject_RichCompareBool(pn, l.obj, op);
+    Py_DECREF(pn);
+    return r;
+}
+
+static inline int int_beyond(PyObject* v, const Limit& l, int op) {
+    if (l.in_c && PyLong_CheckExact(v)) {
+        int overflow = 0;
+        long long x = PyLong_AsLongLongAndOverflow(v, &overflow);
+        if (overflow == 0) return op == Py_GT ? x > l.c : x < l.c;
+        return (op == Py_GT) == (overflow > 0);
+    }
+    return PyObject_RichCompareBool(v, l.obj, op);
+}
+
+static inline int validate(PyObject* obj, const Node* n);
+
+static inline int check_required(PyObject* obj, const Node* n) {
+    for (PyObject* req : n->required) {
+        int has = PyDict_Contains(obj, req);
+        if (has <= 0) return has;
+    }
+    return 1;
+}
+
+static inline int validate_object(PyObject* obj, const Node* n) {
+    if (!PyDict_CheckExact(obj)) return 0;
+    bool props_true = !n->props.empty();
+    if (props_true || n->ap != nullptr) {
+        bool extra_ok = n->ap_present || n->preserve;
+        Py_ssize_t pos = 0;
+        PyObject *k, *v;
+        while (PyDict_Next(obj, &pos, &k, &v)) {
+            const Node* sub = nullptr;
+            if (props_true) {
+                if (!PyUnicode_CheckExact(k)) return 0;
+                sub = find_prop(n, k);
+            }
+            if (sub == nullptr) sub = n->ap;
+            if (sub == nullptr) {
+                if (!extra_ok) return 0;
+                continue;
+            }
+            int r = validate(v, sub);
+            if (r <= 0) return r;
+        }
+    }
+    return check_required(obj, n);
+}
+
+static inline int validate_string(PyObject* obj, const Node* n) {
+    if (!PyUnicode_CheckExact(obj)) return 0;
+    if (n->enum_set != nullptr) {
+        int in = PySequence_Contains(n->enum_set, obj);
+        if (in <= 0) return in;
+    }
+    if (n->search != nullptr) {
+        PyObject* m = PyObject_CallOneArg(n->search, obj);
+        if (m == nullptr) return -1;
+        bool miss = m == Py_None;
+        Py_DECREF(m);
+        if (miss) return 0;
+    }
+    if (n->max_length.present) {
+        int r = len_beyond(PyUnicode_GET_LENGTH(obj), n->max_length, Py_GT);
+        if (r != 0) return r < 0 ? -1 : 0;
+    }
+    if (n->min_length.present) {
+        int r = len_beyond(PyUnicode_GET_LENGTH(obj), n->min_length, Py_LT);
+        if (r != 0) return r < 0 ? -1 : 0;
+    }
+    return 1;
+}
+
+static inline int validate(PyObject* obj, const Node* n) {
+    if (Py_EnterRecursiveCall(" while validating against a CRD schema")) return -1;
+    int r = 1;
+    switch (n->type) {
+    case T_OBJECT:
+        r = validate_object(obj, n);
+        break;
+    case T_ARRAY:
+        if (!PyList_CheckExact(obj)) {
+            r = 0;
+            break;
+        }
+        if (n->max_items.present) {
+            int c = len_beyond(PyList_GET_SIZE(obj), n->max_items, Py_GT);
+            if (c != 0) r = c < 0 ? -1 : 0;
+        }
+        if (n->items != nullptr)
+            for (Py_ssize_t i = 0; r == 1 && i < PyList_GET_SIZE(obj); i++)
+                r = validate(PyList_GET_ITEM(obj, i), n->items);
+        break;
+    case T_STRING:
+        r = validate_string(obj, n);
+        break;
+    case T_INTEGER:
+        if (!PyLong_Check(obj) || PyBool_Check(obj)) {
+            r = 0;
+            break;
+        }
+        if (n->minimum.present) {
+            int c = int_beyond(obj, n->minimum, Py_LT);
+            if (c != 0) r = c < 0 ? -1 : 0;
+        }
+        if (r == 1 && n->maximum.present) {
+            int c = int_beyond(obj, n->maximum, Py_GT);
+            if (c != 0) r = c < 0 ? -1 : 0;
+        }
+        break;
+    case T_BOOLEAN:
+        if (!PyBool_Check(obj)) r = 0;
+        break;
+    case T_NONE:
+    case T_OTHER:
+        break;
+    }
+    if (r == 1 && n->has_any_of) {
+        r = 0;
+        for (const Node* b : n->any_of) {
+            r = validate(obj, b);
+            if (r != 0) break;
+        }
+    }
+    Py_LeaveRecursiveCall();
+    return r;
+}
+
+static inline int validate_changed(PyObject* nw, PyObject* old, const Node* n) {
+    if (nw == old) return 1;
+    if (Py_EnterRecursiveCall(" while validating against a CRD schema")) return -1;
+    int r = 1;
+    if ((PyDict_Check(nw) && !PyDict_CheckExact(nw)) || (PyDict_Check(old) && !PyDict_CheckExact(old)) ||
+        (PyList_Check(nw) && !PyList_CheckExact(nw)) || (PyList_Check(old) && !PyList_CheckExact(old))) {
+        r = 0;
+    } else if (PyDict_CheckExact(nw) && PyDict_CheckExact(old) && n->has_props) {
+        bool extra_ok = n->ap_present || n->preserve;
+        bool props_true = !n->props.empty();
+        Py_ssize_t pos = 0;
+        PyObject *k, *v;
+        while (r == 1 && PyDict_Next(nw, &pos, &k, &v)) {
+            if (!PyUnicode_CheckExact(k)) { r = 0; break; }
+            const Node* sub = find_prop(n, k);
+            if (sub == nullptr) sub = n->ap;
+            if (sub == nullptr) {
+                if (props_true && !extra_ok) r = 0;
+                continue;
+            }
+            PyObject* ov = PyDict_GetItemWithError(old, k);
+            if (ov == nullptr && PyErr_Occurred()) { r = -1; break; }
+            r = ov == nullptr ? validate(v, sub) : validate_changed(v, ov, sub);
+        }
+        if (r == 1) r = check_required(nw, n);
+    } else if (PyList_CheckExact(nw) && PyList_CheckExact(old) && n->items != nullptr) {
+        if (n->max_items.present) {
+            int c = len_beyond(PyList_GET_SIZE(nw), n->max_items, Py_GT);
+            if (c != 0) r = c < 0 ? -1 : 0;
+        }
+        for (Py_ssize_t i = 0; r == 1 && i < PyList_GET_SIZE(nw); i++) {
+            PyObject* item = PyList_GET_ITEM(nw, i);
+            Py_INCREF(item);
+            int seen = 0;
+            for (Py_ssize_t j = 0; seen == 0 && j < PyList_GET_SIZE(old); j++) {
+                PyObject* o = PyList_GET_ITEM(old, j);
+                Py_INCREF(o);
+                seen = PyObject_RichCompareBool(item, o, Py_EQ);
+                Py_DECREF(o);
+            }
+            if (seen < 0) r = -1;
+            else if (seen == 0) r = validate(item, n->items);
+            Py_DECREF(item);
+        }
+    } else {
+        int eq = PyObject_RichCompareBool(nw, old, Py_EQ);
+        if (eq < 0) r = -1;
+        else if (eq == 0) r = validate(nw, n);
+    }
+    Py_LeaveRecursiveCall();
+    return r;
+}
+
+static inline PyObject* dget(PyObject* d, PyObject* key) {
+    PyObject* v = PyDict_GetItemWithError(d, key);
+    if (v == nullptr) PyErr_Clear();
+    return v;
+}
+
+static inline int verdict(const Schema& s, PyObject* nw, PyObject* old) {
+    if (!PyDict_CheckExact(nw)) return 0;
+    PyObject* spec = dget(nw, N.spec);
+    if (old == Py_None) {
+        int r = validate(nw, s.root);
+        if (r <= 0) return r;
+    } else {
+        if (!PyDict_CheckExact(old)) return 0;
+        struct { PyObject* key; const Node* sub; } parts[2] = {{N.spec, s.spec}, {N.status, s.status}};
+        for (auto& part : parts) {
+            PyObject* ns = dget(nw, part.key);
+            PyObject* olds = dget(old, part.key);
+            if (part.sub == nullptr || ns == nullptr || ns == Py_None) continue;
+            int r = validate_changed(ns, olds != nullptr ? olds : Py_None, part.sub);
+            if (r <= 0) return r;
+        }
+        if (s.spec_immutable) {
+            PyObject* ns = spec != nullptr ? spec : Py_None;
+            PyObject* olds = dget(old, N.spec);
+            if (olds == nullptr) olds = Py_None;
+            if (ns != olds) {
+                int ne = PyObject_RichCompareBool(ns, olds, Py_NE);
+                if (ne != 0) return ne < 0 ? -1 : 0;
+            }
+        }
+    }
+    if (spec == nullptr) return 1;
+    int spec_true = PyObject_IsTrue(spec);
+    if (spec_true < 0) return -1;
+    if (!spec_true) return 1;
+    if (!PyDict_CheckExact(spec)) return 0;
+    PyObject* ref = dget(spec, N.nodeClassRef);
+    if (ref == nullptr || !PyDict_Check(ref)) return 1;
+    if (!PyDict_CheckExact(ref)) return 0;
+    PyObject* fields[3] = {N.group, N.kind, N.name};
+    for (PyObject* f : fields) {
+        PyObject* v = dget(ref, f);
+        if (v == nullptr) continue;
+        int eq = PyObject_RichCompareBool(v, N.empty, Py_EQ);
+        if (eq != 0) return eq < 0 ? -1 : 0;
+    }
+    return 1;
+}
+
+
+static inline int apply_defaults(PyObject* obj, const Node* n) {
+    if (!PyDict_Check(obj) || n->props.empty()) return 0;
+    if (Py_EnterRecursiveCall(" while applying CRD defaults")) return -1;
+    bool exact = PyDict_CheckExact(obj);
+    int rc = 0;
+    for (const Prop& p : n->props) {
+        int has = exact ? PyDict_Contains(obj, p.key) : PySequence_Contains(obj, p.key);
+        if (has == 0 && p.node->has_default) {
+            PyObject* value = p.node->default_value;
+            if ((exact ? PyDict_SetItem(obj, p.key, value) : PyObject_SetItem(obj, p.key, value)) < 0)
+                has = -1;
+            else
+                has = exact ? 1 : PySequence_Contains(obj, p.key);
+        }
+        if (has < 0) { rc = -1; break; }
+        if (has == 0) continue;
+        PyObject* v;
+        if (exact) {
+            v = PyDict_GetItemWithError(obj, p.key);
+            Py_XINCREF(v);
+        } else {
+            v = PyObject_GetItem(obj, p.key);
+        }
+        if (v == nullptr) { rc = -1; break; }
+        if (PyDict_Check(v)) {
+            rc = apply_defaults(v, p.node);
+        } else if (PyList_Check(v) && p.node->items != nullptr) {
+            if (PyList_CheckExact(v)) {
+                for (Py_ssize_t i = 0; rc == 0 && i < PyList_GET_SIZE(v); i++) {
+                    PyObject* item = PyList_GET_ITEM(v, i);
+                    Py_INCREF(item);
+                    rc = apply_defaults(item, p.node->items);
+                    Py_DECREF(item);
+                }
+            } else {
+                PyObject* it = PyObject_GetIter(v);
+                PyObject* item;
+                if (it == nullptr) rc = -1;
+                while (rc == 0 && (item = PyIter_Next(it)) != nullptr) {
+                    rc = apply_defaults(item, p.node->items);
+                    Py_DECREF(item);
+                }
+                if (rc == 0 && PyErr_Occurred()) rc = -1;
+                Py_XDECREF(it);
+            }
+        }
+        Py_DECREF(v);
+        if (rc < 0) break;
+    }
+    Py_LeaveRecursiveCall();
+    return rc;
+}
+
+}
+
+#endif
diff --git a/native/jsontree.cpp b/native/jsontree.cpp
--- a/native/jsontree.cpp
+++ b/native/jsontree.cpp
@@ -1,6 +1,7 @@
 #define PY_SSIZE_T_CLEAN
 #include <Python.h>
 
+#include "crdschema_walk.h"
 #include "jsontree_walk.h"
 
 namespace {
@@ -30,323 +31,46 @@
 }
 
 
-struct Names {
-    PyObject *type, *properties, *additionalProperties, *preserve, *required, *items,
-        *maxItems, *enum_set, *enum_, *pattern_re, *pattern, *maxLength, *minLength,
-        *minimum, *maximum, *anyOf, *search, *spec, *status, *nodeClassRef, *group,
-        *kind, *name, *empty;
-} S;
-
-inline PyObject* sget(PyObject* schema, PyObject* key) {
-    PyObject* v = PyDict_GetItemWithError(schema, key);
-    if (v == nullptr) PyErr_Clear();
-    return v;
+PyObject* py_crd_compile(PyObject*, PyObject* const* args, Py_ssize_t nargs) {
+    if (nargs != 2) {
+        PyErr_SetString(PyExc_TypeError, "crd_compile(schema, spec_immutable) takes 2 arguments");
+        return nullptr;
+    }
+    int imm = PyObject_IsTrue(args[1]);
+    if (imm < 0) return nullptr;
+    PyObject* capsule = crdschema_walk::compile_capsule(args[0], imm != 0);
+    if (capsule == nullptr && !PyErr_Occurred()) Py_RETURN_NONE;
+    return capsule;
 }
 
-inline PyObject* sget2(PyObject* schema, PyObject* overlay, PyObject* key) {
-    if (overlay != nullptr) {
-        PyObject* v = sget(overlay, key);
-        if (v != nullptr) return v;
+PyObject* verdict_bool(int r) {
+    if (r < 0) {
+        PyErr_Clear();
+        r = 0;
     }
-    return sget(schema, key);
+    return PyBool_FromLong(r);
 }
 
-inline bool is_str(PyObject* o, const char* s) {
-    return o != nullptr && PyUnicode_CheckExact(o) && PyUnicode_CompareWithASCIIString(o, s) == 0;
+PyObject* py_crd_valid_compiled(PyObject*, PyObject* const* args, Py_ssize_t nargs) {
+    const crdschema_walk::Schema* s = nargs == 3 ? crdschema_walk::from_capsule(args[0]) : nullptr;
+    if (s == nullptr) {
+        PyErr_SetString(PyExc_TypeError,
+                        "crd_valid_compiled(compiled, new, old_or_None) takes a crd_compile "
+                        "capsule and 2 more arguments");
+        return nullptr;
+    }
+    return verdict_bool(crdschema_walk::verdict(*s, args[1], args[2]));
 }
 
-int len_cmp(Py_ssize_t n, PyObject* limit, int op) {
-    PyObject* pn = PyLong_FromSsize_t(n);
-    if (pn == nullptr) return -1;
-    int r = PyObject_RichCompareBool(pn, limit, op);
-    Py_DECREF(pn);
-    return r;
-}
-
-int validate(PyObject* obj, PyObject* schema, PyObject* overlay);
-
-int validate_changed(PyObject* nw, PyObject* old, PyObject* schema);
-
-int check_required(PyObject* obj, PyObject* schema) {
-    PyObject* req = sget(schema, S.required);
-    if (req == nullptr) return 1;
-    if (!PyList_CheckExact(req) && !PyTuple_CheckExact(req)) return 0;
-    Py_ssize_t n = PySequence_Fast_GET_SIZE(req);
-    for (Py_ssize_t i = 0; i < n; i++) {
-        int has = PyDict_Contains(obj, PySequence_Fast_GET_ITEM(req, i));
-        if (has <= 0) return has;
+PyObject* py_crd_defaults(PyObject*, PyObject* const* args, Py_ssize_t nargs) {
+    const crdschema_walk::Schema* s = nargs == 2 ? crdschema_walk::from_capsule(args[0]) : nullptr;
+    if (s == nullptr) {
+        PyErr_SetString(PyExc_TypeError,
+                        "crd_defaults(compiled, obj) takes a crd_compile capsule and 1 more argument");
+        return nullptr;
     }
-    return 1;
-}
-
-int validate_string(PyObject* obj, PyObject* schema, PyObject* overlay) {
-    if (!PyUnicode_Check(obj)) return 0;
-    if (!PyUnicode_CheckExact(obj)) return 0;
-    PyObject* enum_set = sget2(schema, overlay, S.enum_set);
-    if (enum_set != nullptr && enum_set != Py_None) {
-        int in = PySequence_Contains(enum_set, obj);
-        if (in <= 0) return in;
-    } else {
-        PyObject* en = sget2(schema, overlay, S.enum_);
-        if (en != nullptr) {
-            int in = PySequence_Contains(en, obj);
-            if (in <= 0) return in;
-        }
-    }
-    PyObject* pat = sget2(schema, overlay, S.pattern_re);
-    if (pat != nullptr && pat != Py_None) {
-        PyObject* m = PyObject_CallMethodOneArg(pat, S.search, obj);
-        if (m == nullptr) return -1;
-        bool miss = m == Py_None;
-        Py_DECREF(m);
-        if (miss) return 0;
-    } else if (sget2(schema, overlay, S.pattern) != nullptr) {
-        return 0;
-    }
-    PyObject* lim = sget2(schema, overlay, S.maxLength);
-    if (lim != nullptr) {
-        int r = len_cmp(PyUnicode_GET_LENGTH(obj), lim, Py_GT);
-        if (r != 0) return r < 0 ? -1 : 0;
-    }
-    lim = sget2(schema, overlay, S.minLength);
-    if (lim != nullptr) {
-        int r = len_cmp(PyUnicode_GET_LENGTH(obj), lim, Py_LT);
-        if (r != 0) return r < 0 ? -1 : 0;
-    }
-    return 1;
-}
-
-int validate_object(PyObject* obj, PyObject* schema) {
-    if (!PyDict_Check(obj)) return 0;
-    if (!PyDict_CheckExact(obj)) return 0;
-    PyObject* props = sget(schema, S.properties);
-    PyObject* ap = sget(schema, S.additionalProperties);
-    if (ap == Py_None) ap = nullptr;
-    if (ap != nullptr && PyDict_Check(ap) && !PyDict_CheckExact(ap)) return 0;
-    bool ap_schema = ap != nullptr && PyDict_CheckExact(ap);
-    int props_true = props == nullptr ? 0 : PyObject_IsTrue(props);
-    if (props_true < 0) return -1;
-    if (props_true && !PyDict_CheckExact(props)) return 0;
-    if (props_true || ap_schema) {
-        bool extra_ok = ap != nullptr;
-        if (props_true && !extra_ok) {
-            PyObject* pu = sget(schema, S.preserve);
-            int t = pu == nullptr ? 0 : PyObject_IsTrue(pu);
-            if (t < 0) return -1;
-            extra_ok = t != 0;
-        }
-        Py_ssize_t pos = 0;
-        PyObject *k, *v;
-        while (PyDict_Next(obj, &pos, &k, &v)) {
-            PyObject* sub = nullptr;
-            if (props_true) {
-                sub = PyDict_GetItemWithError(props, k);
-                if (sub == nullptr && PyErr_Occurred()) return -1;
-                if (sub == Py_None) sub = nullptr;
-            }
-            if (sub == nullptr && ap_schema) sub = ap;
-            if (sub == nullptr) {
-                if (!extra_ok) return 0;
-                continue;
-            }
-            if (!PyDict_CheckExact(sub)) return 0;
-            int r = validate(v, sub, nullptr);
-            if (r <= 0) return r;
-        }
-    }
-    return check_required(obj, schema);
-}
-
-int validate_any_of(PyObject* obj, PyObject* schema, PyObject* branches) {
-    if (!PyList_CheckExact(branches)) return 0;
-    bool string_fields = sget(schema, S.pattern) || sget(schema, S.pattern_re) ||
-                         sget(schema, S.maxLength) || sget(schema, S.minLength) ||
-                         sget(schema, S.enum_);
-    for (Py_ssize_t i = 0; i < PyList_GET_SIZE(branches); i++) {
-        PyObject* b = PyList_GET_ITEM(branches, i);
-        if (!PyDict_CheckExact(b)) return 0;
-        PyObject* overlay = nullptr;
-        if (string_fields && is_str(sget(b, S.type), "string")) overlay = schema;
-        int r = validate(obj, b, overlay);
-        if (r != 0) return r;
-    }
-    return 0;
-}
-
-int validate(PyObject* obj, PyObject* schema, PyObject* overlay) {
-    if (Py_EnterRecursiveCall(" while validating against a CRD schema")) return -1;
-    int r = 1;
-    PyObject* t = sget(schema, S.type);
-    if (t != nullptr && t != Py_None && !PyUnicode_CheckExact(t)) {
-        r = 0;
-    } else if (is_str(t, "object") ||
-               ((t == nullptr || t == Py_None) && sget(schema, S.properties) != nullptr)) {
-        r = validate_object(obj, schema);
-    } else if (is_str(t, "array")) {
-        if (!PyList_CheckExact(obj)) {
-            r = 0;
-        } else {
-            PyObject* lim = sget(schema, S.maxItems);
-            if (lim != nullptr) {
-                int c = len_cmp(PyList_GET_SIZE(obj), lim, Py_GT);
-                if (c != 0) r = c < 0 ? -1 : 0;
-            }
-            PyObject* items = sget(schema, S.items);
-            int items_true = (r == 1 && items != nullptr) ? PyObject_IsTrue(items) : 0;
-            if (items_true < 0) r = -1;
-            if (r == 1 && items_true) {
-                if (!PyDict_CheckExact(items)) r = 0;
-                for (Py_ssize_t i = 0; r == 1 && i < PyList_GET_SIZE(obj); i++)
-                    r = validate(PyList_GET_ITEM(obj, i), items, nullptr);
-            }
-        }
-    } else if (is_str(t, "string")) {
-        r = validate_string(obj, schema, overlay);
-    } else if (is_str(t, "integer")) {
-        if (!PyLong_Check(obj) || PyBool_Check(obj)) {
-            r = 0;
-        } else {
-            PyObject* lim = sget(schema, S.minimum);
-            if (lim != nullptr) {
-                int c = PyObject_RichCompareBool(obj, lim, Py_LT);
-                if (c != 0) r = c < 0 ? -1 : 0;
-            }
-            lim = sget(schema, S.maximum);
-            if (r == 1 && lim != nullptr) {
-                int c = PyObject_RichCompareBool(obj, lim, Py_GT);
-                if (c != 0) r = c < 0 ? -1 : 0;
-            }
-        }
-    } else if (is_str(t, "boolean")) {
-        if (!PyBool_Check(obj)) r = 0;
-    }
-    if (r == 1) {
-        PyObject* any_of = sget(schema, S.anyOf);
-        if (any_of != nullptr)
-            r = overlay != nullptr ? 0 : validate_any_of(obj, schema, any_of);
-    }
-    Py_LeaveRecursiveCall();
-    return r;
-}
-
-int validate_changed(PyObject* nw, PyObject* old, PyObject* schema) {
-    if (nw == old) return 1;
-    if (Py_EnterRecursiveCall(" while validating against a CRD schema")) return -1;
-    int r = 1;
-    PyObject* props = sget(schema, S.properties);
-    if (props == Py_None) props = nullptr;
-    PyObject* items = sget(schema, S.items);
-    if ((PyDict_Check(nw) && !PyDict_CheckExact(nw)) || (PyDict_Check(old) && !PyDict_CheckExact(old)) ||
-        (PyList_Check(nw) && !PyList_CheckExact(nw)) || (PyList_Check(old) && !PyList_CheckExact(old)) ||
-        (props != nullptr && !PyDict_CheckExact(props)) ||
-        (items != nullptr && PyDict_Check(items) && !PyDict_CheckExact(items))) {
-        r = 0;
-    } else if (PyDict_CheckExact(nw) && PyDict_CheckExact(old) && props != nullptr) {
-        PyObject* ap = sget(schema, S.additionalProperties);
-        if (ap == Py_None) ap = nullptr;
-        bool ap_schema = ap != nullptr && PyDict_CheckExact(ap);
-        if (ap != nullptr && PyDict_Check(ap) && !ap_schema) r = 0;
-        bool extra_ok = ap != nullptr;
-        if (r == 1 && !extra_ok) {
-            PyObject* pu = sget(schema, S.preserve);
-            int t = pu == nullptr ? 0 : PyObject_IsTrue(pu);
-            if (t < 0) r = -1;
-            extra_ok = t > 0;
-        }
-        bool props_true = PyDict_GET_SIZE(props) > 0;
-        Py_ssize_t pos = 0;
-        PyObject *k, *v;
-        while (r == 1 && PyDict_Next(nw, &pos, &k, &v)) {
-            PyObject* sub = PyDict_GetItemWithError(props, k);
-            if (sub == nullptr && PyErr_Occurred()) { r = -1; break; }
-            if (sub == Py_None) sub = nullptr;
-            if (sub == nullptr && ap_schema) sub = ap;
-            if (sub == nullptr) {
-                if (props_true && !extra_ok) r = 0;
-                continue;
-            }
-            if (!PyDict_CheckExact(sub)) { r = 0; break; }
-            PyObject* ov = PyDict_GetItemWithError(old, k);
-            if (ov == nullptr && PyErr_Occurred()) { r = -1; break; }
-            r = ov == nullptr ? validate(v, sub, nullptr) : validate_changed(v, ov, sub);
-        }
-        if (r == 1) r = check_required(nw, schema);
-    } else if (PyList_CheckExact(nw) && PyList_CheckExact(old) && items != nullptr &&
-               PyDict_CheckExact(items)) {
-        PyObject* lim = sget(schema, S.maxItems);
-        if (lim != nullptr) {
-            int c = len_cmp(PyList_GET_SIZE(nw), lim, Py_GT);
-            if (c != 0) r = c < 0 ? -1 : 0;
-        }
-        for (Py_ssize_t i = 0; r == 1 && i < PyList_GET_SIZE(nw); i++) {
-            PyObject* item = PyList_GET_ITEM(nw, i);
-            Py_INCREF(item);
-            int seen = 0;
-            for (Py_ssize_t j = 0; seen == 0 && j < PyList_GET_SIZE(old); j++) {
-                PyObject* o = PyList_GET_ITEM(old, j);
-                Py_INCREF(o);
-                seen = PyObject_RichCompareBool(item, o, Py_EQ);
-                Py_DECREF(o);
-            }
-            if (seen < 0) r = -1;
-            else if (seen == 0) r = validate(item, items, nullptr);
-            Py_DECREF(item);
-        }
-    } else {
-        int eq = PyObject_RichCompareBool(nw, old, Py_EQ);
-        if (eq < 0) r = -1;
-        else if (eq == 0) r = validate(nw, schema, nullptr);
-    }
-    Py_LeaveRecursiveCall();
-    return r;
-}
-
-int crd_valid(PyObject* schema, PyObject* nw, PyObject* old, bool spec_immutable) {
-    if (!PyDict_CheckExact(schema) || !PyDict_CheckExact(nw)) return 0;
-    PyObject* spec = sget(nw, S.spec);
-    if (old == Py_None) {
-        int r = validate(nw, schema, nullptr);
-        if (r <= 0) return r;
-    } else {
-        if (!PyDict_CheckExact(old)) return 0;
-        PyObject* props = sget(schema, S.properties);
-        if (props != nullptr && !PyDict_CheckExact(props)) return 0;
-        PyObject* keys[2] = {S.spec, S.status};
-        for (PyObject* key : keys) {
-            PyObject* ns = sget(nw, key);
-            PyObject* olds = sget(old, key);
-            PyObject* sub = props ? sget(props, key) : nullptr;
-            if (sub == nullptr || sub == Py_None || ns == nullptr || ns == Py_None) continue;
-            if (!PyDict_CheckExact(sub)) return 0;
-            int r = validate_changed(ns, olds ? olds : Py_None, sub);
-            if (r <= 0) return r;
-        }
-        if (spec_immutable) {
-            PyObject* ns = spec ? spec : Py_None;
-            PyObject* olds = sget(old, S.spec);
-            if (olds == nullptr) olds = Py_None;
-            if (ns != olds) {
-                int ne = PyObject_RichCompareBool(ns, olds, Py_NE);
-                if (ne != 0) return ne < 0 ? -1 : 0;
-            }
-        }
-    }
-    if (spec == nullptr) return 1;
-    int spec_true = PyObject_IsTrue(spec);
-    if (spec_true < 0) return -1;
-    if (!spec_true) return 1;
-    if (!PyDict_CheckExact(spec)) return 0;
-    PyObject* ref = sget(spec, S.nodeClassRef);
-    if (ref == nullptr || !PyDict_Check(ref)) return 1;
-    if (!PyDict_CheckExact(ref)) return 0;
-    PyObject* fields[3] = {S.group, S.kind, S.name};
-    for (PyObject* f : fields) {
-        PyObject* v = sget(ref, f);
-        if (v == nullptr) continue;
-        int eq = PyObject_RichCompareBool(v, S.empty, Py_EQ);
-        if (eq != 0) return eq < 0 ? -1 : 0;
-    }
-    return 1;
+    if (crdschema_walk::apply_defaults(args[1], s->root) < 0) return nullptr;
+    Py_RETURN_NONE;
 }
 
 PyObject* py_crd_valid(PyObject*, PyObject* const* args, Py_ssize_t nargs) {
@@ -357,12 +81,9 @@
     }
     int imm = PyObject_IsTrue(args[3]);
     if (imm < 0) return nullptr;
-    int r = crd_valid(args[0], args[1], args[2], imm != 0);
-    if (r < 0) {
-        PyErr_Clear();
-        r = 0;
-    }
-    return PyBool_FromLong(r);
+    std::unique_ptr<crdschema_walk::Schema> s = crdschema_walk::compile(args[0], imm != 0);
+    if (s == nullptr) Py_RETURN_FALSE;
+    return verdict_bool(crdschema_walk::verdict(*s, args[1], args[2]));
 }
 
 PyMethodDef methods[] = {
@@ -376,6 +97,13 @@
     {"crd_valid", (PyCFunction)(void (*)(void))py_crd_valid, METH_FASTCALL,
      "crd_valid(schema, new, old_or_None, spec_immutable): True when CRDValidator "
      "would report no violation."},
+    {"crd_compile", (PyCFunction)(void (*)(void))py_crd_compile, METH_FASTCALL,
+     "crd_compile(schema, spec_immutable): the compiled schema as a capsule, or None "
+     "for a schema the native walks do not mirror."},
+    {"crd_valid_compiled", (PyCFunction)(void (*)(void))py_crd_valid_compiled, METH_FASTCALL,
+     "crd_valid_compiled(compiled, new, old_or_None): crd_valid over a crd_compile capsule."},
+    {"crd_defaults", (PyCFunction)(void (*)(void))py_crd_defaults, METH_FASTCALL,
+     "crd_defaults(compiled, obj): fill the schema's defaults into obj, in place."},
     {nullptr, nullptr, 0, nullptr},
 };
 
@@ -386,38 +114,8 @@
 };
 
 bool intern_names() {
-    struct { PyObject** slot; const char* text; } table[] = {
-        {&str_metadata, "metadata"},
-        {&S.type, "type"},
-        {&S.properties, "properties"},
-        {&S.additionalProperties, "additionalProperties"},
-        {&S.preserve, "x-kubernetes-preserve-unknown-fields"},
-        {&S.required, "required"},
-        {&S.items, "items"},
-        {&S.maxItems, "maxItems"},
-        {&S.enum_set, "_enum_set"},
-        {&S.enum_, "enum"},
-        {&S.pattern_re, "_pattern_re"},
-        {&S.pattern, "pattern"},
-        {&S.maxLength, "maxLength"},
-        {&S.minLength, "minLength"},
-        {&S.minimum, "minimum"},
-        {&S.maximum, "maximum"},
-        {&S.anyOf, "anyOf"},
-        {&S.search, "search"},
-        {&S.spec, "spec"},
-        {&S.status, "status"},
-        {&S.nodeClassRef, "nodeClassRef"},
-        {&S.group, "group"},
-        {&S.kind, "kind"},
-        {&S.name, "name"},
-        {&S.empty, ""},
-    };
-    for (auto& e : table) {
-        *e.slot = PyUnicode_InternFromString(e.text);
-        if (*e.slot == nullptr) return false;
-    }
-    return true;
+    str_metadata = PyUnicode_InternFromString("metadata");
+    return str_metadata != nullptr && crdschema_walk::init_names();
 }
 
 }
diff --git a/native/revstore.cpp b/native/revstore.cpp
--- a/native/revstore.cpp
+++ b/native/revstore.cpp
@@ -3,6 +3,7 @@
 
 #include <limits.h>
 
+#include "crdschema_walk.h"
 #include "jsontree_walk.h"
 
 namespace {
@@ -15,12 +16,14 @@
     PyObject *metadata, *name, *namespace_, *uid, *creationTimestamp, *generation,
         *deletionTimestamp, *finalizers, *resourceVersion, *spec, *status, *empty, *Event,
         *ADDED, *MODIFIED, *DELETED, *rv_attr, *history_attr, *watchers_attr, *append,
-        *put_nowait;
+        *put_nowait, *compiled, *native_valid;
 } S;
 
 PyObject* long_one;
 PyObject* uuid4_str;
 PyObject* now_rfc3339;
+PyObject* validator_type;
+PyObject* crdschema_globals;
 
 struct Ref {
     PyObject* p;
@@ -109,8 +112,27 @@
     return 1;
 }
 
+const crdschema_walk::Schema* compiled_schema(PyObject* validator, Ref& hold) {
+    if (validator_type == nullptr || (PyObject*)Py_TYPE(validator) != validator_type) return nullptr;
+    PyObject* on = PyDict_GetItemWithError(crdschema_globals, S.native_valid);
+    if (on == nullptr || on == Py_None) {
+        PyErr_Clear();
+        return nullptr;
+    }
+    hold.reset(PyObject_GetAttr(validator, S.compiled));
+    if (hold == nullptr) PyErr_Clear();
+    return crdschema_walk::from_capsule(hold);
+}
+
 int valid(PyObject* validator, PyObject* nw, PyObject* old) {
     if (validator == Py_None) return 1;
+    Ref capsule;
+    if (const crdschema_walk::Schema* schema = compiled_schema(validator, capsule)) {
+        int r = old == Py_None ? crdschema_walk::apply_defaults(nw, schema->root) : 0;
+        if (r == 0) r = crdschema_walk::verdict(*schema, nw, old);
+        if (r < 0) PyErr_Clear();
+        return r > 0;
+    }
     PyObject* args[2] = {nw, old};
     Ref errs(PyObject_Vectorcall(validator, args, 2, nullptr));
     if (errs == nullptr) return -1;
@@ -478,11 +500,25 @@
     Py_RETURN_NONE;
 }
 
+PyObject* py_set_admission(PyObject*, PyObject* const* args, Py_ssize_t nargs) {
+    if (nargs != 2 || !PyType_Check(args[0]) || !PyDict_CheckExact(args[1])) {
+        PyErr_SetString(PyExc_TypeError,
+                        "set_admission(validator_type, module_dict) takes a type and a dict");
+        return nullptr;
+    }
+    Py_XSETREF(validator_type, newref(args[0]));
+    Py_XSETREF(crdschema_globals, newref(args[1]));
+    Py_RETURN_NONE;
+}
+
 #define FAST(f) (PyCFunction)(void (*)(void))f, METH_FASTCALL
 
 PyMethodDef methods[] = {
     {"set_helpers", FAST(py_set_helpers),
      "set_helpers(uuid4_str, now_rfc3339): bind the uid and clock functions create and delete call."},
+    {"set_admission", FAST(py_set_admission),
+     "set_admission(validator_type, module_dict): bind CRDValidator and the dict holding its "
+     "_native_valid switch; such a validator's compiled schema is then walked inside the verbs."},
     {"get", FAST(py_get), "get(bucket, namespace, name): a copy of the stored revision."},
     {"create", FAST(py_create),
      "create(server, gvk, bucket, obj, validator, event_cap): store a new object, return a copy."},
@@ -527,13 +563,15 @@
         {&S.watchers_attr, "_watchers"},
         {&S.append, "append"},
         {&S.put_nowait, "put_nowait"},
+        {&S.compiled, "_compiled"},
+        {&S.native_valid, "_native_valid"},
     };
     for (auto& e : table) {
         *e.slot = PyUnicode_InternFromString(e.text);
         if (*e.slot == nullptr) return false;
     }
     long_one = PyLong_FromLong(1);
-    return long_one != nullptr;
+    return long_one != nullptr && crdschema_walk::init_names();
 }
 
 }
```

Measured after the change: 108,500 NodeClaims/min. 0.958x the previous value.
